# musket-ml/segmentation_training_pipeline

Hardware: AMD Instinct MI355X
Metric: images/sec U-Net/ResNet34 512x512 bs16 training step (higher is better)
Workload: dtype bf16; 1 GPU; U-Net/ResNet34 512x512x3 1-class, batch 16 per GPU, BCE+Dice, Adam, on-device augment S1 (BASELINE.json configs[1]); global_batch=16, parallelism=dp1, hipgraph=True

## Files before the change

### include/stp_hip.h

```cpp
#ifndef STP_HIP_H
#define STP_HIP_H

#include <stddef.h>
#include <stdint.h>

#ifdef __cplusplus
extern "C" {
#endif

#define STP_OK 0
#define STP_E_BADARG (-1)
#define STP_E_LAUNCH (-2)
#define STP_E_WORKSPACE (-3)

#define STP_F32 0
#define STP_BF16 1
#define STP_F16 3

#define STP_SRC_DIRECT 0
#define STP_SRC_NEAREST2X 1
#define STP_SRC_ZEROINS2X 2

int stp_abi_version(void);
int stp_storage_dtype(void);
// ... 83 lines not shown
  const float* src_bn_gamma;
  const float* src_bn_beta;
  int32_t src_bn_relu;
} stp_wgrad_params;

size_t stp_conv2d_wgrad_workspace_bytes(const stp_wgrad_params* p);
int stp_conv2d_wgrad(const stp_wgrad_params* p, void* workspace, size_t workspace_bytes, void* stream);
int stp_conv2d_wgrad_partial(const stp_wgrad_params* p, void* workspace, size_t workspace_bytes, int32_t variant, void* stream);
int stp_conv2d_wgrad_reduce(const stp_wgrad_params* p, const void* workspace, int32_t variant, void* stream);
int stp_wgrad_sc_eligible(const stp_wgrad_params* p);
int stp_wgrad_sc_slabs(const stp_wgrad_params* p);
int stp_wgrad_sc_partial(const stp_wgrad_params* p, void* workspace, void* stream);
int stp_conv2d_wgrad_kernel_id(const stp_wgrad_params* p);

int stp_wgrad_group_class(const stp_wgrad_params* p);
size_t stp_wgrad_group_table_bytes(const stp_wgrad_params* const* layers, int32_t n);
size_t stp_wgrad_group_workspace_bytes(const stp_wgrad_params* const* layers, int32_t n);
int stp_wgrad_group_build(const stp_wgrad_params* const* layers, int32_t n, void* host_table, size_t table_bytes);
int stp_wgrad_group_partial(const void* host_table, const void* dev_table, void* workspace, size_t workspace_bytes, void* stream);
int stp_wgrad_group_reduce(const void* host_table, const void* dev_table, const void* workspace, void* stream);

int stp_weight_prepare(const float* master, void* fwd, void* bwd, int32_t Cout, int32_t KH, int32_t KW,
                       int32_t Cin, int32_t KWp, int32_t Cinp, int32_t CoutB, int32_t dtype, void* stream);
size_t stp_weight_prepare_desc_bytes(void);
int64_t stp_weight_prepare_desc_fill(void* desc_host, int32_t index, int64_t start, const float* master, void* fwd, void* bwd,
                                     int32_t Cout, int32_t KH, int32_t KW, int32_t Cin, int32_t KWp, int32_t Cinp, int32_t CoutB);
int stp_weight_prepare_batched(const void* desc_dev, int32_t nlayers, int64_t total, int32_t dtype, void* stream);
int stp_weight_grad_unpad(const float* padded, float* grad, int32_t Cout, int32_t KH, int32_t KW,
                          int32_t Cin, int32_t KWp, int32_t Cinp, int32_t accumulate, void* stream);
int stp_stem_beta_grad(const float* padded_dw, const float* master, float* dbeta, int32_t Cout, int32_t KH,
                       int32_t KW, int32_t Cin, int32_t KWp, int32_t Cinp, int32_t one_ch, void* stream);

#define STP_U8 2
size_t stp_bn_workspace_bytes(int32_t C);
int stp_bn_apply_slots(const void* x, void* y, int32_t dtype, int64_t rows, int32_t C, const int64_t* slots, int32_t nslots,
                       float eps, float momentum, float* mean, float* rstd, float* moving_mean, float* moving_var,
                       const float* gamma, const float* beta, int32_t relu, void* stream);
int stp_bn_backward_slots(const void* x, const void* g, void* dx, int32_t dtype, int64_t rows, int32_t C, const float* mean,
                          const float* rstd, const float* gamma, const int64_t* slots, int32_t nslots, float* dgamma,
                          float* dbeta, int32_t accumulate_dx, void* stream);
int stp_zero_bytes(void* p, int64_t bytes, void* stream);
int stp_bn_backward_fused(const void* x, const void* g, void* dx, int32_t dtype, int64_t rows, int32_t C,
                          const float* mean, const float* rstd, const float* gamma, const float* partial, int32_t tiles,
                          float* dgamma, float* dbeta, int32_t accumulate_dx, void* workspace, size_t workspace_bytes,
                          void* stream);
int stp_bn_finalize_apply_ok(int32_t dtype, int64_t rows, int32_t C, int32_t tiles);
int stp_bn_finalize_apply(const float* partial, int32_t tiles, const void* x, void* y, int32_t dtype, int64_t rows, int32_t C,
                          float eps, float momentum, float* mean, float* rstd, float* moving_mean, float* moving_var,
                          const float* gamma, const float* beta, int32_t relu, void* stream);
int stp_bn_backward_fused_add(const void* x, const void* g, void* dx, const void* dadd, int32_t dtype, int64_t rows, int32_t C,
                              const float* mean, const float* rstd, const float* gamma, const float* partial, int32_t tiles,
                              float* dgamma, float* dbeta, int32_t accumulate_dx, void* workspace, size_t workspace_bytes,
                              void* stream);
int stp_bn_stats(const void* x, int32_t xdtype, int64_t rows, int32_t C, float eps, float momentum,
                 float* mean, float* rstd, float* moving_mean, float* moving_var,
                 void* workspace, size_t workspace_bytes, void* stream);
int stp_bn_finalize(const float* partial, int32_t tiles, int64_t rows, int32_t C, float eps, float momentum,
                    float* mean, float* rstd, float* moving_mean, float* moving_var, void* stream);
int stp_bn_apply(const void* x, int32_t xdtype, void* y, int32_t ydtype, int64_t rows, int32_t C, int32_t Cy,
                 const float* mean, const float* rstd, const float* gamma, const float* beta,
                 int32_t relu, float pad_value, void* stream);
int stp_bn_inference(const void* x, int32_t xdtype, void* y, int32_t ydtype, int64_t rows, int32_t C, int32_t Cy,
                     const float* moving_mean, const float* moving_var, float eps,
                     const float* gamma, const float* beta, int32_t relu, float pad_value, void* stream);
int stp_bn_backward(const void* x, const void* dy, void* dx, int32_t dtype, int64_t rows, int32_t C,
                    const float* mean, const float* rstd, const float* gamma, const float* beta,
                    float* dgamma, float* dbeta, int32_t relu, int32_t accumulate_dx,
                    void* workspace, size_t workspace_bytes, void* stream);

int stp_maxpool3x3s2(const void* x, void* y, uint8_t* idx, int32_t N, int32_t H, int32_t W, int32_t C,
                     int32_t dtype, void* stream);
int stp_maxpool3x3s2_bwd(const uint8_t* idx, const void* dy, void* dx, int32_t N, int32_t H, int32_t W, int32_t C,
                         int32_t dtype, int32_t accumulate, void* stream);
int stp_bn_apply_maxpool3x3s2(const void* x, void* yb, void* y, uint8_t* idx, int32_t N, int32_t H, int32_t W, int32_t C, int32_t dtype,
                              const float* mean, const float* rstd, const float* gamma, const float* beta, int32_t relu, void* stream);
int stp_maxpool3x3s2_bwd_bn_tiles(int32_t N, int32_t H, int32_t W, int32_t C, int32_t dtype);
int stp_maxpool3x3s2_bwd_bn(const uint8_t* idx, const void* dy, void* dx, int32_t N, int32_t H, int32_t W, int32_t C, int32_t dtype,
                            int32_t accumulate, const void* bn_x, const float* mean, const float* rstd, const float* gamma,
                            const float* beta, int32_t relu, float* partial, void* stream);
int stp_maxpool2x2(const void* x, void* y, uint8_t* idx, int32_t N, int32_t H, int32_t W, int32_t C, int32_t dtype, void* stream);
int stp_maxpool2x2_bwd(const uint8_t* idx, const void* dy, void* dx, int32_t N, int32_t H, int32_t W, int32_t C, int32_t dtype,
                       int32_t accumulate, void* stream);
size_t stp_avgpool_workspace_bytes(int32_t N, int32_t H, int32_t W, int32_t C, int32_t k);
int stp_avgpool(const void* x, void* y, int32_t N, int32_t H, int32_t W, int32_t C, int32_t k, int32_t dtype, void* workspace,
                size_t workspace_bytes, void* stream);
int stp_avgpool_bwd(const void* dy, void* dx, int32_t N, int32_t H, int32_t W, int32_t C, int32_t k, int32_t dtype,
                    int32_t accumulate, void* stream);
int stp_avgpool_pyramid_ok(int32_t N, int32_t H, int32_t W, int32_t C, int32_t k0, int32_t k1, int32_t k2, int32_t k3, int32_t dtype);
size_t stp_avgpool_pyramid_workspace_bytes(int32_t N, int32_t H, int32_t W, int32_t C, int32_t k0, int32_t dtype);
int stp_avgpool_pyramid(const void* x, void* y0, void* y1, void* y2, void* y3, int32_t k0, int32_t k1, int32_t k2, int32_t k3, int32_t N,
                        int32_t H, int32_t W, int32_t C, int32_t dtype, void* workspace, size_t workspace_bytes, void* stream);
int stp_avgpool_pyramid_bwd(const void* dy0, const void* dy1, const void* dy2, const void* dy3, int32_t k0, int32_t k1, int32_t k2, int32_t k3,
                            void* dx, int32_t N, int32_t H, int32_t W, int32_t C, int32_t dtype, int32_t accumulate, void* stream);
int stp_maxpool_k(const void* x, void* y, int32_t* idx, int32_t N, int32_t H, int32_t W, int32_t C, int32_t k, int32_t dtype, void* stream);
int stp_maxpool_k_bwd(const int32_t* idx, const void* dy, void* dx, int32_t N, int32_t H, int32_t W, int32_t C, int32_t k, int32_t dtype,
                      int32_t accumulate, void* stream);
int stp_relu_bwd(const void* y, void* dy, int64_t count, int32_t dtype, void* stream);

int stp_upsample2x_bwd(const void* dy, void* dx, int32_t N, int32_t H, int32_t W, int32_t C, int32_t ldy,
                       int32_t dtype, int32_t accumulate, void* stream);
int stp_tapsum_fwd(const void* z, void* y, const float* bias, int32_t N, int32_t H, int32_t W, int32_t Cout, int32_t Zc, int32_t Cy, int32_t dtype,
                   void* stream);
int stp_tapsum_bwd(const void* dy, void* dz, int32_t N, int32_t H, int32_t W, int32_t Cout, int32_t Cdy, int32_t Cdz, int32_t dtype, void* stream);
int stp_scatter2x_bwd(const void* t, void* dx, int32_t N, int32_t H, int32_t W, int32_t C, int32_t dtype, int32_t accumulate, void* stream);
int stp_scatter2x_bwd_bn_tiles(int32_t N, int32_t H, int32_t W, int32_t C, int32_t dtype);
int stp_scatter2x_bwd_bn(const void* t, void* dx, int32_t N, int32_t H, int32_t W, int32_t C, int32_t dtype, int32_t accumulate,
// ... 225 lines not shown
```

### segmentation_training_pipeline_amd/_lib.py

```python
import ctypes as C
import os

HERE = os.path.dirname(os.path.abspath(__file__))
LIB_PATH = os.environ.get("STP_LIB") or os.path.join(HERE, "libstp_hip.so")

LIB_F16_PATH = os.environ.get("STP_LIB_F16") or os.path.join(HERE, "libstp_hip_f16.so")

F32, BF16, U8, F16 = 0, 1, 2, 3
SRC_DIRECT, SRC_NEAREST2X, SRC_ZEROINS2X = 0, 1, 2

vp, i32, i64, f32, sz = C.c_void_p, C.c_int32, C.c_int64, C.c_float, C.c_size_t


class StpError(RuntimeError):
    pass


class ConvParams(C.Structure):
    _fields_ = [("src0", vp), ("src1", vp), ("weight", vp), ("bias", vp), ("residual", vp), ("dst0", vp), ("dst1", vp),
                ("N", i32), ("Hs0", i32), ("Ws0", i32), ("Hv", i32), ("Wv", i32), ("C0", i32), ("C1", i32),
                ("src0_mode", i32), ("KH", i32), ("KW", i32), ("stride", i32), ("pad", i32),
                ("Ho", i32), ("Wo", i32), ("Cout", i32), ("Cd0", i32),
                ("accumulate0", i32), ("accumulate1", i32), ("relu", i32), ("dtype", i32), ("tile", i32),
                ("stats_tiles", i32), ("stats_partial", vp),
# ... 31 lines not shown
    "stp_conv2d_scw": (i32, [C.POINTER(ConvParams), vp]),
    "stp_conv2d_scw_eligible": (i32, [C.POINTER(ConvParams)]),
    "stp_conv2d_scw_stats_tiles": (i32, [C.POINTER(ConvParams)]),
    "stp_conv2d_scn": (i32, [C.POINTER(ConvParams), vp]),
    "stp_conv2d_scn_eligible": (i32, [C.POINTER(ConvParams)]),
    "stp_conv2d_scn_stats_tiles": (i32, [C.POINTER(ConvParams)]),
    "stp_conv2d_s64": (i32, [C.POINTER(ConvParams), vp]),
    "stp_conv2d_s64_eligible": (i32, [C.POINTER(ConvParams)]),
    "stp_conv2d_s64_stats_tiles": (i32, [C.POINTER(ConvParams)]),
    "stp_conv2d_pw_eligible": (i32, [C.POINTER(ConvParams)]),
    "stp_conv2d_pw_cols": (i32, [C.POINTER(ConvParams)]),
    "stp_conv2d_pw": (i32, [C.POINTER(ConvParams), vp]),
    "stp_conv2d_stem_eligible": (i32, [C.POINTER(ConvParams)]),
    "stp_conv2d_stem": (i32, [C.POINTER(ConvParams), vp]),
    "stp_conv2d_halo_variant": (i32, [C.POINTER(ConvParams)]),
    "stp_conv2d_halo_tiles": (i32, [C.POINTER(ConvParams), i32]),
    "stp_conv2d_halo": (i32, [C.POINTER(ConvParams), i32, vp]),
    "stp_conv2d_wgrad_workspace_bytes": (sz, [C.POINTER(WgradParams)]),
    "stp_conv2d_wgrad": (i32, [C.POINTER(WgradParams), vp, sz, vp]),
    "stp_conv2d_wgrad_partial": (i32, [C.POINTER(WgradParams), vp, sz, i32, vp]),
    "stp_conv2d_wgrad_reduce": (i32, [C.POINTER(WgradParams), vp, i32, vp]),
    "stp_wgrad_reduce_desc_bytes": (sz, []),
    "stp_wgrad_reduce_desc_fill": (i64, [vp, i32, C.POINTER(WgradParams), vp]),
    "stp_wgrad_reduce_batched": (i32, [vp, i32, i64, vp]),
    "stp_wgrad_sc_eligible": (i32, [C.POINTER(WgradParams)]),
    "stp_wgrad_sc_slabs": (i32, [C.POINTER(WgradParams)]),
    "stp_wgrad_sc_partial": (i32, [C.POINTER(WgradParams), vp, vp]),
    "stp_conv2d_wgrad_kernel_id": (i32, [C.POINTER(WgradParams)]),
    "stp_wgrad_group_class": (i32, [C.POINTER(WgradParams)]),
    "stp_wgrad_group_table_bytes": (sz, [vp, i32]),
    "stp_wgrad_group_workspace_bytes": (sz, [vp, i32]),
    "stp_wgrad_group_build": (i32, [vp, i32, vp, sz]),
    "stp_wgrad_group_partial": (i32, [vp, vp, vp, sz, vp]),
    "stp_wgrad_group_reduce": (i32, [vp, vp, vp, vp]),
    "stp_weight_prepare": (i32, [vp, vp, vp, i32, i32, i32, i32, i32, i32, i32, i32, vp]),
    "stp_weight_prepare_desc_bytes": (sz, []),
    "stp_weight_prepare_desc_fill": (i64, [vp, i32, i64, vp, vp, vp, i32, i32, i32, i32, i32, i32, i32]),
    "stp_weight_prepare_batched": (i32, [vp, i32, i64, i32, vp]),
    "stp_weight_grad_unpad": (i32, [vp, vp, i32, i32, i32, i32, i32, i32, i32, vp]),
    "stp_stem_beta_grad": (i32, [vp, vp, vp, i32, i32, i32, i32, i32, i32, i32, vp]),
    "stp_bn_workspace_bytes": (sz, [i32]),
    "stp_bn_stats": (i32, [vp, i32, i64, i32, f32, f32, vp, vp, vp, vp, vp, sz, vp]),
    "stp_bn_finalize": (i32, [vp, i32, i64, i32, f32, f32, vp, vp, vp, vp, vp]),
    "stp_bn_apply": (i32, [vp, i32, vp, i32, i64, i32, i32, vp, vp, vp, vp, i32, f32, vp]),
    "stp_bn_inference": (i32, [vp, i32, vp, i32, i64, i32, i32, vp, vp, f32, vp, vp, i32, f32, vp]),
    "stp_bn_backward": (i32, [vp, vp, vp, i32, i64, i32, vp, vp, vp, vp, vp, vp, i32, i32, vp, sz, vp]),
    "stp_bn_apply_slots": (i32, [vp, vp, i32, i64, i32, vp, i32, f32, f32, vp, vp, vp, vp, vp, vp, i32, vp]),
    "stp_bn_backward_slots": (i32, [vp, vp, vp, i32, i64, i32, vp, vp, vp, vp, i32, vp, vp, i32, vp]),
    "stp_zero_bytes": (i32, [vp, i64, vp]),
    "stp_bn_backward_fused": (i32, [vp, vp, vp, i32, i64, i32, vp, vp, vp, vp, i32, vp, vp, i32, vp, sz, vp]),
    "stp_bn_finalize_apply_ok": (i32, [i32, i64, i32, i32]),
    "stp_bn_finalize_apply": (i32, [vp, i32, vp, vp, i32, i64, i32, f32, f32, vp, vp, vp, vp, vp, vp, i32, vp]),
    "stp_bn_backward_fused_add": (i32, [vp, vp, vp, vp, i32, i64, i32, vp, vp, vp, vp, i32, vp, vp, i32, vp, sz, vp]),
    "stp_maxpool3x3s2": (i32, [vp, vp, vp, i32, i32, i32, i32, i32, vp]),
    "stp_maxpool3x3s2_bwd": (i32, [vp, vp, vp, i32, i32, i32, i32, i32, i32, vp]),
    "stp_bn_apply_maxpool3x3s2": (i32, [vp, vp, vp, vp, i32, i32, i32, i32, i32, vp, vp, vp, vp, i32, vp]),
    "stp_maxpool3x3s2_bwd_bn_tiles": (i32, [i32, i32, i32, i32, i32]),
    "stp_maxpool3x3s2_bwd_bn": (i32, [vp, vp, vp, i32, i32, i32, i32, i32, i32, vp, vp, vp, vp, vp, i32, vp, vp]),
    "stp_maxpool2x2": (i32, [vp, vp, vp, i32, i32, i32, i32, i32, vp]),
    "stp_maxpool2x2_bwd": (i32, [vp, vp, vp, i32, i32, i32, i32, i32, i32, vp]),
    "stp_avgpool_workspace_bytes": (sz, [i32, i32, i32, i32, i32]),
    "stp_avgpool": (i32, [vp, vp, i32, i32, i32, i32, i32, i32, vp, sz, vp]),
    "stp_avgpool_bwd": (i32, [vp, vp, i32, i32, i32, i32, i32, i32, i32, vp]),
    "stp_avgpool_pyramid_ok": (i32, [i32, i32, i32, i32, i32, i32, i32, i32, i32]),
    "stp_avgpool_pyramid_workspace_bytes": (sz, [i32, i32, i32, i32, i32, i32]),
    "stp_avgpool_pyramid": (i32, [vp, vp, vp, vp, vp, i32, i32, i32, i32, i32, i32, i32, i32, i32, vp, sz, vp]),
    "stp_avgpool_pyramid_bwd": (i32, [vp, vp, vp, vp, i32, i32, i32, i32, vp, i32, i32, i32, i32, i32, i32, vp]),
    "stp_maxpool_k": (i32, [vp, vp, vp, i32, i32, i32, i32, i32, i32, vp]),
    "stp_maxpool_k_bwd": (i32, [vp, vp, vp, i32, i32, i32, i32, i32, i32, i32, vp]),
    "stp_relu_bwd": (i32, [vp, vp, i64, i32, vp]),
    "stp_upsample2x_bwd": (i32, [vp, vp, i32, i32, i32, i32, i32, i32, i32, vp]),
    "stp_tapsum_fwd": (i32, [vp, vp, vp, i32, i32, i32, i32, i32, i32, i32, vp]),
    "stp_tapsum_bwd": (i32, [vp, vp, i32, i32, i32, i32, i32, i32, i32, vp]),
    "stp_scatter2x_bwd": (i32, [vp, vp, i32, i32, i32, i32, i32, i32, vp]),
    "stp_scatter2x_bwd_bn_tiles": (i32, [i32, i32, i32, i32, i32]),
    "stp_scatter2x_bwd_bn": (i32, [vp, vp, i32, i32, i32, i32, i32, i32, vp, vp, vp, vp, vp, i32, vp, vp]),
    "stp_upsample2x_bwd_bn_tiles": (i32, [i32, i32, i32, i32, i32, i32]),
    "stp_upsample2x_bwd_bn": (i32, [vp, vp, i32, i32, i32, i32, i32, i32, i32, vp, vp, vp, vp, vp, i32, vp, vp]),
    "stp_upsample2x_add": (i32, [vp, vp, i32, i32, i32, i32, i32, vp]),
    "stp_resize_bilinear": (i32, [vp, vp, i32, i32, i32, i32, i32, i32, i32, i32, vp]),
    "stp_upsample_sum": (i32, [vp, vp, vp, vp, i32, i32, i32, i32, vp, i32, i32, i32, i32, i32, vp]),
    "stp_copy_cols_f32": (i32, [vp, i32, vp, i32, i32, i32, i32, vp]),
    "stp_resize_bilinear_bwd_workspace_bytes": (sz, [i32, i32, i32, i32, i32]),
    "stp_resize_bilinear_bwd": (i32, [vp, vp, i32, i32, i32, i32, i32, i32, i32, i32, i32, vp, sz, vp]),
    "stp_resize_nearest": (i32, [vp, vp, i32, i32, i32, i32, i32, i32, i32, i32, vp]),
    "stp_resize_nearest_bwd": (i32, [vp, vp, i32, i32, i32, i32, i32, i32, i32, i32, i32, vp]),
    "stp_channel_sum": (i32, [vp, i32, i64, i32, vp, i32, vp, sz, vp]),
    "stp_add_inplace": (i32, [vp, vp, i64, i32, vp]),
    "stp_loss_workspace_bytes": (sz, []),
    "stp_sigmoid_bce_dice": (i32, [vp, vp, i64, i32, f32, f32, vp, vp, i32, f32, vp, sz, vp]),
    "stp_sigmoid_loss_ex": (i32, [vp, vp, i64, i32, vp, vp, vp, i32, f32, vp, sz, vp]),
    "stp_sigmoid_loss_bias_grad": (i32, [vp, i64, vp, i32, vp]),
    "stp_sigmoid_multilabel_loss": (i32, [vp, vp, i64, i32, i32, i32, vp, vp, vp, i32, f32, vp, sz, vp]),
    "stp_sigmoid_multilabel_bias_grad": (i32, [vp, i64, i32, vp, i32, vp]),
    "stp_softmax_loss_ex": (i32, [vp, vp, i64, i32, i32, i32, vp, vp, vp, i32, f32, vp, sz, vp]),
    "stp_softmax_loss_masked": (i32, [vp, vp, i64, i32, i32, i32, vp, vp, vp, i32, f32, vp, sz, i32, vp, vp]),
    "stp_lovasz_workspace_bytes": (sz, [i64, i32]),
    "stp_lovasz_hinge": (i32, [vp, vp, i32, i64, i32, f32, vp, vp, i32, vp, sz, vp]),
    "stp_sigmoid": (i32, [vp, vp, i64, i32, vp]),
    "stp_softmax_cce_dice": (i32, [vp, vp, i64, i32, i32, i32, f32, f32, vp, vp, i32, f32, vp, sz, vp]),
    "stp_softmax_cce_dice_up_ok": (i32, [i32, i32, i32]),
    "stp_softmax_cce_dice_up_corner_bytes": (sz, [i32, i32, i32, i32]),
    "stp_softmax_cce_dice_up": (i32, [vp, vp, i32, i32, i32, i32, i32, i32, i32, f32, f32, vp, vp, i32, f32, vp, vp, vp, sz, vp, sz, vp]),
    "stp_softmax": (i32, [vp, vp, i64, i32, i32, i32, vp]),
    "stp_class_confusion_workspace_bytes": (sz, [i32]),
    "stp_class_confusion": (i32, [vp, vp, i64, i32, i32, i32, vp, vp, sz, vp]),
# ... 132 lines not shown
```

### segmentation_training_pipeline_amd/csrc/bn_pool.hip

```cpp
#include "common.h"
#include <algorithm>
#include <cstdlib>

#define BN_MAX_BLOCKS 1024
#ifndef POOL_ROWS
#define POOL_ROWS 4
#endif


template <typename T> __device__ __forceinline__ f32x4 ld4(const T* p);
template <> __device__ __forceinline__ f32x4 ld4<float>(const float* p) { return load4(p); }
template <> __device__ __forceinline__ f32x4 ld4<bf16_t>(const bf16_t* p) { return load4(p); }

template <typename T, int V> __device__ __forceinline__ void ldv(const T* p, float (&o)[V]) {
  if constexpr (V == 4) {
    const f32x4 v = ld4<T>(p);
    o[0] = v.x; o[1] = v.y; o[2] = v.z; o[3] = v.w;
  } else {
    const u32x4 r = *reinterpret_cast<const u32x4*>(p);
#pragma unroll
    for (int e = 0; e < 4; ++e) { o[2 * e] = h16lo_to_f32(r[e]); o[2 * e + 1] = h16hi_to_f32(r[e]); }
  }
}
template <typename T, int V> __device__ __forceinline__ void stv(T* p, const float (&o)[V]) {
// ... 1014 lines not shown
      const float xhl = (xl - mu[2 * e]) * rs[2 * e], xhh = (xh_ - mu[2 * e + 1]) * rs[2 * e + 1];
      float ol = sc[2 * e] * (gl - k1[2 * e] - xhl * k2[2 * e]), oh = sc[2 * e + 1] * (gh - k1[2 * e + 1] - xhh * k2[2 * e + 1]);
      if (dadd) { ol += h16lo_to_f32(dr[e]); oh += h16hi_to_f32(dr[e]); }
      o[e] = pack_bf16x2(ol, oh);
    }
    *reinterpret_cast<u32x4*>(dx + off) = o;
  };
  if (pre) {
#pragma unroll
    for (int k = 0; k < 4; ++k) one((size_t)(r + 32 * k) * C + col, px[k], pg[k], pd[k]);
    r += 128;
  }
  for (; r + 96 < rb; r += 128) {
    u32x4 vx[4], vg[4], vd[4] = {z4, z4, z4, z4};
#pragma unroll
    for (int k = 0; k < 4; ++k) {
      const size_t o = (size_t)(r + 32 * k) * C + col;
      vx[k] = *reinterpret_cast<const u32x4*>(x + o);
      vg[k] = *reinterpret_cast<const u32x4*>(g + o);
      if (dadd) vd[k] = *reinterpret_cast<const u32x4*>(dadd + o);
    }
#pragma unroll
    for (int k = 0; k < 4; ++k) one((size_t)(r + 32 * k) * C + col, vx[k], vg[k], vd[k]);
  }
  for (; r < rb; r += 32) {
    const size_t o = (size_t)r * C + col;
    const u32x4 vx = *reinterpret_cast<const u32x4*>(x + o), vg = *reinterpret_cast<const u32x4*>(g + o);
    const u32x4 vd = dadd ? *reinterpret_cast<const u32x4*>(dadd + o) : z4;
    one(o, vx, vg, vd);
  }
}

static int bn_bwd_fused_launch(const void* x, const void* g, void* dx, const void* dadd, int64_t rows, int C, const float* mean, const float* rstd,
                               const float* gamma, const float* partial, int tiles, float* dgamma, float* dbeta, int accumulate_dx, hipStream_t s) {
  const int chunks = bn_fused_chunks(rows, C);
  hipLaunchKernelGGL(bn_bwd_finalize_apply_kernel, dim3((C / BNF_SLAB) * chunks), dim3(256), 0, s, partial, tiles, (const bf16_t*)x, (const bf16_t*)g,
                     (bf16_t*)dx, accumulate_dx ? (const bf16_t*)dadd : (const bf16_t*)nullptr, rows, C, chunks, (float)(1.0 / (double)rows), mean, rstd,
                     gamma, dgamma, dbeta);
  STP_LAUNCH_CHECK();
  return STP_OK;
}

__global__ __launch_bounds__(256) void bn_bwd_finalize_tiles_kernel(const float* __restrict__ partial, int tiles, int C, float* sums,
                                                                    float* dgamma, float* dbeta) {
  __shared__ double sh[2][4];
  const int c = blockIdx.x;
  double S, Q;
  bnf_channel_sums(partial + (size_t)c * tiles, partial + ((size_t)C + c) * tiles, tiles, sh, S, Q);
  if (threadIdx.x != 0) return;
  sums[c] = (float)S;
  sums[C + c] = (float)Q;
  if (dbeta) dbeta[c] = (float)S;
  if (dgamma) dgamma[c] = (float)Q;
}

extern "C" int stp_bn_backward_slots(const void* x, const void* g, void* dx, int32_t dtype, int64_t rows, int32_t C, const float* mean,
                                     const float* rstd, const float* gamma, const int64_t* slots, int32_t nslots, float* dgamma,
                                     float* dbeta, int32_t accumulate_dx, void* stream) {
  if (!stp_dtype_ok(dtype)) return STP_E_BADARG;
  if (!x || !g || !dx || !mean || !rstd || !slots || rows <= 0 || C <= 0 || (C & 3) || nslots < 1 || (nslots & (nslots - 1))) return STP_E_BADARG;
  hipStream_t s = (hipStream_t)stream;
  const bool v8 = dtype == STP_H16 && (C & 7) == 0;
  const size_t lds2 = 6 * (size_t)C * sizeof(float);
  const int gr = grid_fixed_channels(grid_for_amortised(rows * (C / (v8 ? 8 : 4)), 8), C / (v8 ? 8 : 4));
  const float inv_rows = (float)(1.0 / (double)rows);
  const long long* sl = (const long long*)slots;
  if (v8)
    hipLaunchKernelGGL((bn_bwd_apply_kernel<bf16_t, 8>), dim3(gr), dim3(256), lds2, s, (const bf16_t*)x, (const bf16_t*)g, (bf16_t*)dx, rows, C,
                       mean, rstd, gamma, (const float*)nullptr, (const float*)nullptr, inv_rows, 0, accumulate_dx, sl, nslots, dgamma, dbeta);
  else if (dtype == STP_H16)
    hipLaunchKernelGGL((bn_bwd_apply_kernel<bf16_t, 4>), dim3(gr), dim3(256), lds2, s, (const bf16_t*)x, (const bf16_t*)g, (bf16_t*)dx, rows, C,
                       mean, rstd, gamma, (const float*)nullptr, (const float*)nullptr, inv_rows, 0, accumulate_dx, sl, nslots, dgamma, dbeta);
  else if (dtype == STP_F32)
    hipLaunchKernelGGL((bn_bwd_apply_kernel<float, 4>), dim3(gr), dim3(256), lds2, s, (const float*)x, (const float*)g, (float*)dx, rows, C,
                       mean, rstd, gamma, (const float*)nullptr, (const float*)nullptr, inv_rows, 0, accumulate_dx, sl, nslots, dgamma, dbeta);
  else
    return STP_E_BADARG;
  STP_LAUNCH_CHECK();
  return STP_OK;
}

extern "C" int stp_bn_backward_fused_add(const void* x, const void* g, void* dx, const void* dadd, int32_t dtype, int64_t rows, int32_t C,
                                     const float* mean, const float* rstd, const float* gamma, const float* partial,
                                     int32_t tiles, float* dgamma, float* dbeta, int32_t accumulate_dx, void* workspace,
                                     size_t workspace_bytes, void* stream) {
  if (!stp_dtype_ok(dtype)) return STP_E_BADARG;
  if (!x || !g || !dx || (accumulate_dx && !dadd) || !mean || !rstd || !partial || !workspace || rows <= 0 || C <= 0 || (C & 3) || tiles <= 0) return STP_E_BADARG;
  if (workspace_bytes < stp_bn_workspace_bytes(C)) return STP_E_WORKSPACE;
  hipStream_t s = (hipStream_t)stream;
  if (bn_fused_ok(dtype, rows, C, tiles))
    return bn_bwd_fused_launch(x, g, dx, dadd, rows, C, mean, rstd, gamma, partial, tiles, dgamma, dbeta, accumulate_dx, s);
  float* sums = (float*)workspace + (size_t)(BN_MAX_BLOCKS - 1) * 2 * C;
  hipLaunchKernelGGL(bn_bwd_finalize_tiles_kernel, dim3(C), dim3(256), 0, s, partial, tiles, C, sums, dgamma, dbeta);
  STP_LAUNCH_CHECK();
  const bool v8 = dtype == STP_H16 && (C & 7) == 0;
  const size_t lds2 = 6 * (size_t)C * sizeof(float);
  const int gr = grid_fixed_channels(grid_for_amortised(rows * (C / (v8 ? 8 : 4)), 8), C / (v8 ? 8 : 4));
  const float inv_rows = (float)(1.0 / (double)rows);
  if (v8)
    hipLaunchKernelGGL((bn_bwd_apply_kernel<bf16_t, 8>), dim3(gr), dim3(256), lds2, s, (const bf16_t*)x, (const bf16_t*)g,
                       (bf16_t*)dx, rows, C, mean, rstd, gamma, (const float*)nullptr, sums, inv_rows, 0, accumulate_dx, (const long long*)nullptr, 0, (float*)nullptr, (float*)nullptr,
                       (const bf16_t*)dadd);
  else if (dtype == STP_H16)
    hipLaunchKernelGGL((bn_bwd_apply_kernel<bf16_t, 4>), dim3(gr), dim3(256), lds2, s, (const bf16_t*)x, (const bf16_t*)g,
                       (bf16_t*)dx, rows, C, mean, rstd, gamma, (const float*)nullptr, sums, inv_rows, 0, accumulate_dx, (const long long*)nullptr, 0, (float*)nullptr, (float*)nullptr,
                       (const bf16_t*)dadd);
// ... 1889 lines not shown
```

### segmentation_training_pipeline_amd/csrc/conv_sc.h

```cpp
#pragma once
#include "common.h"
#include <cstdlib>
#include <type_traits>
#include <utility>

struct ScArgs {
  const char* src;
  const char* weight;
  const float* bias;
  char* dst;
  int N, H, W, Hs, Ws, Cout, up, accumulate, relu;
  int tiles_x, tiles_y;
  FastDiv divTx, divTy;
  float* stats;
  int stat_slots;
  BnBack bnb;
  int sum2;
  uint32_t src_bytes;
  BnBack pbn;
};

template <typename T> struct ScStageBn;
template <> struct ScStageBn<float> {
  f32x4 sc, sh;
  __device__ __forceinline__ void load(const BnBack& b, int c) { const BnBackCh k = bnback_load(b, c); sc = k.sc; sh = k.sh; }
  __device__ __forceinline__ void load_tab(const float* tsc, const float* tsh, int c) {
    sc = *reinterpret_cast<const f32x4*>(tsc + c); sh = *reinterpret_cast<const f32x4*>(tsh + c);
  }
  __device__ __forceinline__ u32x4 apply(const u32x4& r, int relu) const {
    u32x4 o;
#pragma unroll
    for (int e = 0; e < 4; ++e) o[e] = __float_as_uint(bn_act(bn_affine(__uint_as_float(r[e]), sc[e], sh[e]), relu));
    return o;
  }
};
template <> struct ScStageBn<bf16_t> {
  f32x2 sc[4], sh[4];
  __device__ __forceinline__ void load(const BnBack& b, int c) {
    const BnBackCh k0 = bnback_load(b, c), k1 = bnback_load(b, c + 4);
    sc[0] = f32x2{k0.sc[0], k0.sc[1]}; sc[1] = f32x2{k0.sc[2], k0.sc[3]}; sc[2] = f32x2{k1.sc[0], k1.sc[1]}; sc[3] = f32x2{k1.sc[2], k1.sc[3]};
    sh[0] = f32x2{k0.sh[0], k0.sh[1]}; sh[1] = f32x2{k0.sh[2], k0.sh[3]}; sh[2] = f32x2{k1.sh[0], k1.sh[1]}; sh[3] = f32x2{k1.sh[2], k1.sh[3]};
  }
  __device__ __forceinline__ void load_tab(const float* tsc, const float* tsh, int c) {
#pragma unroll
    for (int e = 0; e < 4; ++e) { sc[e] = *reinterpret_cast<const f32x2*>(tsc + c + 2 * e); sh[e] = *reinterpret_cast<const f32x2*>(tsh + c + 2 * e); }
  }
  __device__ __forceinline__ u32x4 apply(const u32x4& r, int relu) const {
    u32x4 o;
#pragma unroll
    for (int e = 0; e < 4; ++e) {
      f32x2 v = {h16lo_to_f32(r[e]), h16hi_to_f32(r[e])};
      v = __builtin_elementwise_fma(v, sc[e], sh[e]);
      o[e] = pack_bf16x2(bn_act(v.x, relu), bn_act(v.y, relu));
    }
    return o;
  }
};


constexpr int SC_TH = 8, SC_TW = 32, SC_HW = SC_TW + 2, SC_HH = SC_TH + 2;

template <int... Ks, typename F>
__device__ __forceinline__ void sc_unroll_seq(std::integer_sequence<int, Ks...>, F&& f) { (f(std::integral_constant<int, Ks>{}), ...); }
template <int N, typename F>
__device__ __forceinline__ void sc_unroll(F&& f) { sc_unroll_seq(std::make_integer_sequence<int, N>{}, f); }
#ifndef SC_RING
#define SC_RING 8
#endif

#ifndef SC_WPE_SMALL
#define SC_WPE_SMALL 4
#endif

static inline bool sc_stream_on() {
  static const bool on = !(getenv("STP_SC_STREAM") && atoi(getenv("STP_SC_STREAM")) == 0);
  return on;
}
static inline int sc_cu_count() {
  static const int cus = [] {
    int d = 0, n = 0;
    if (hipGetDevice(&d) != hipSuccess || hipDeviceGetAttribute(&n, hipDeviceAttributeMultiprocessorCount, d) != hipSuccess || n <= 0) n = 256;
    return n;
  }();
  return cus;
}
static inline int sc_stream_blocks(int dtype, int cin, int cout, int ntiles) {
  const int per_cu = cout <= 16 ? (dtype == STP_H16 && cin <= 16 ? SC_WPE_SMALL : 3) : 2;
  const int64_t b = (int64_t)sc_cu_count() * per_cu;
  return (int)(b < ntiles ? b : ntiles);
}


struct ScWgArgs {
  const char* src;
  const char* dy;
  float* slabs;
  int N, H, W, Hs, Ws, Cout, up;
  int tiles_x, tiles_y, ntiles;
  int ctot, coff;
  uint32_t src_bytes, dy_bytes;
  BnBack pbn;
};

constexpr int ST_HH = (SC_TH - 1) * 2 + 7, ST_HW = 70, ST_WROW = 464, ST_HALO = ST_HH * ST_HW * 8, ST_WBYTES = 64 * ST_WROW;

struct StemArgs {
  const char* src;
  const char* weight;
  char* dst;
  int N, H, W, Ho, Wo, tiles_x, tiles_y;
  FastDiv divTx, divTy;
  float* stats;
  uint32_t src_bytes;
};

bool stem_lean_serves(int N, int H, int W);
int stem_lean_blocks(int ntiles);
int stem_lean_launch(const StemArgs& a, hipStream_t s);
bool stem_wg_lean_serves(int N, int H, int W, int Ho, int Wo);
int stem_wg_lean_blocks(int N, int Ho, int Wo);
int stem_wg_lean_launch(const void* src, const void* dy, float* slabs, int N, int H, int W, int Ho, int Wo, hipStream_t s);

int sc_lean_launch(const ScArgs& a, int cin, int dtype, hipStream_t s);
int sc_wg_lean_launch(const ScWgArgs& a, int cin, int cout, int dtype, int blocks, hipStream_t s);
```

### segmentation_training_pipeline_amd/csrc/conv_sc.hip

```cpp
#include "conv_sc.h"

__device__ __forceinline__ f32x4 sc_stored(f32x4 v, const float*) { return v; }
__device__ __forceinline__ f32x4 sc_stored(f32x4 v, const bf16_t*) {
  const uint32_t a = pack_bf16x2(v.x, v.y), b = pack_bf16x2(v.z, v.w);
  return f32x4{h16lo_to_f32(a), h16hi_to_f32(a), h16lo_to_f32(b), h16hi_to_f32(b)};
}

template <typename T> struct ScMma;
template <> struct ScMma<bf16_t> {
  __device__ static __forceinline__ void run(const u32x4& a, const u32x4& b, f32x4& c) {
    c = mfma16_16x16x32(a, b, c);
  }
};
template <> struct ScMma<float> {
  __device__ static __forceinline__ void run(const u32x4& a, const u32x4& b, f32x4& c) {
    c = __builtin_amdgcn_mfma_f32_16x16x4f32(__uint_as_float(a.x), __uint_as_float(b.x), c, 0, 0, 0);
    c = __builtin_amdgcn_mfma_f32_16x16x4f32(__uint_as_float(a.y), __uint_as_float(b.y), c, 0, 0, 0);
    c = __builtin_amdgcn_mfma_f32_16x16x4f32(__uint_as_float(a.z), __uint_as_float(b.z), c, 0, 0, 0);
    c = __builtin_amdgcn_mfma_f32_16x16x4f32(__uint_as_float(a.w), __uint_as_float(b.w), c, 0, 0, 0);
  }
};

template <typename T> struct ScRaw4;
template <> struct ScRaw4<float> {
// ... 481 lines not shown
  ep.reset_stats();
  for (int tile = t_first; tile < t_end; tile += 2 * t_step) {
    body(tile, std::integral_constant<int, 0>{});
    if (tile + t_step < t_end) body(tile + t_step, std::integral_constant<int, 1>{});
  }
  ep.flush_stats(a, red, (int)blockIdx.x, (int)gridDim.x, tid, wave, lr, lg);
}

template <typename T, int CIN, int TM>
static int launch_sc(const ScArgs& a, hipStream_t s) {
  const int ntiles = a.N * a.tiles_x * a.tiles_y;
  if (sc_stream_on()) {
    constexpr int NV = SC_HH * SC_HW * (CIN / Elem<T>::VEC), NPASS = (NV + 255) / 256;
    const size_t lds = (size_t)2 * NPASS * 4096 + (4 * TM * 16 * 2 + 128 + 64) * sizeof(float);
    const int blocks = sc_stream_blocks(Elem<T>::DTYPE, CIN, TM * 16, ntiles);
    static bool attr_set = false;
    if (lds > 64 * 1024 && !attr_set) {
      if (hipFuncSetAttribute(reinterpret_cast<const void*>(conv_sc_stream_kernel<T, CIN, TM>), hipFuncAttributeMaxDynamicSharedMemorySize, (int)lds) != hipSuccess)
        return STP_E_LAUNCH;
      attr_set = true;
    }
    hipLaunchKernelGGL((conv_sc_stream_kernel<T, CIN, TM>), dim3(blocks), dim3(256), lds, s, a);
    STP_LAUNCH_CHECK();
    return STP_OK;
  }
  const size_t lds = (size_t)SC_HH * SC_HW * CIN * sizeof(T) + 4 * TM * 16 * 2 * sizeof(float);
  hipLaunchKernelGGL((conv_sc_kernel<T, CIN, TM>), dim3(ntiles), dim3(256), lds, s, a);
  STP_LAUNCH_CHECK();
  return STP_OK;
}

extern "C" int stp_conv2d_sc_stats_tiles(const stp_conv_params* p) {
  const int ntiles = p->N * ceil_div(p->Hv, SC_TH) * ceil_div(p->Wv, SC_TW);
  if (!sc_stream_on() || p->stats_slots) return ntiles;
  return sc_stream_blocks(p->dtype, p->C0, p->Cout <= 16 ? 16 : 32, ntiles);
}

template <typename T>
static int dispatch_sc(const ScArgs& a, int cin, hipStream_t s) {
  const int tm = a.Cout <= 16 ? 1 : 2;
  switch (cin * 4 + tm) {
    case 4 * 4 + 1: if constexpr (sizeof(T) == 4) return launch_sc<T, 4, 1>(a, s); else return STP_E_BADARG;
    case 4 * 4 + 2: if constexpr (sizeof(T) == 4) return launch_sc<T, 4, 2>(a, s); else return STP_E_BADARG;
    case 8 * 4 + 1: return launch_sc<T, 8, 1>(a, s);
    case 8 * 4 + 2: return launch_sc<T, 8, 2>(a, s);
    case 16 * 4 + 1: return launch_sc<T, 16, 1>(a, s);
    case 16 * 4 + 2: return launch_sc<T, 16, 2>(a, s);
    case 32 * 4 + 1: return launch_sc<T, 32, 1>(a, s);
    case 32 * 4 + 2: return launch_sc<T, 32, 2>(a, s);
    default: return STP_E_BADARG;
  }
}

extern "C" int stp_conv2d_sc_eligible(const stp_conv_params* p) {
  if (!p || !stp_dtype_ok(p->dtype)) return 0;
  const int vec = p->dtype == STP_H16 ? 8 : 4;
  const int cin = p->C0;
  const bool cin_ok = p->dtype == STP_F32 ? (cin == 4 || cin == 8 || cin == 16) : (cin == 8 || cin == 16 || cin == 32);
  return p->KH == 3 && p->KW == 3 && p->stride == 1 && p->pad == 1 && p->C1 == 0 && cin_ok && (cin % vec) == 0 && p->Cout <= 32 &&
         p->Cd0 == p->Cout && !p->residual && p->Ho == p->Hv && p->Wo == p->Wv &&
         (p->src0_mode == STP_SRC_DIRECT || (p->src0_mode == STP_SRC_NEAREST2X && p->Hv == 2 * p->Hs0 && p->Wv == 2 * p->Ws0));
}

extern "C" int stp_conv2d_sc(const stp_conv_params* p, void* stream) {
  if (!stp_conv2d_sc_eligible(p) || !p->src0 || !p->weight || !p->dst0) return STP_E_BADARG;
  ScArgs a;
  a.src = (const char*)p->src0; a.weight = (const char*)p->weight; a.bias = p->bias; a.dst = (char*)p->dst0;
  a.N = p->N; a.H = p->Hv; a.W = p->Wv; a.Hs = p->Hs0; a.Ws = p->Ws0; a.Cout = p->Cout;
  a.up = p->src0_mode == STP_SRC_NEAREST2X; a.accumulate = p->accumulate0; a.relu = p->relu;
  {
    const uint64_t sb = (uint64_t)p->N * p->Hs0 * p->Ws0 * p->C0 * (p->dtype == STP_H16 ? 2 : 4);
    if (sb >= 0x80000000ull) return STP_E_BADARG;
    a.src_bytes = (uint32_t)sb;
  }
  a.tiles_x = ceil_div(a.W, SC_TW); a.tiles_y = ceil_div(a.H, SC_TH);
  a.divTx = make_fastdiv((uint32_t)a.tiles_x); a.divTy = make_fastdiv((uint32_t)a.tiles_y);
  a.stats = p->stats_partial;
  a.stat_slots = p->stats_slots;
  if (a.stats && (p->Cout & 3)) return STP_E_BADARG;
  if (a.stat_slots && (!a.stats || (a.stat_slots & (a.stat_slots - 1)) || a.stat_slots > 64)) return STP_E_BADARG;
  a.bnb.x = (const char*)p->bnb_x; a.bnb.mean = p->bnb_mean; a.bnb.rstd = p->bnb_rstd; a.bnb.gamma = p->bnb_gamma;
  a.bnb.beta = p->bnb_beta; a.bnb.relu = p->bnb_relu;
  a.sum2 = p->dst_sum2x2;
  a.pbn.x = nullptr; a.pbn.mean = p->src_bn_mean; a.pbn.rstd = p->src_bn_rstd; a.pbn.gamma = p->src_bn_gamma; a.pbn.beta = p->src_bn_beta;
  a.pbn.relu = p->src_bn_relu;
  if (a.pbn.mean && !a.pbn.rstd) return STP_E_BADARG;
  if (a.bnb.x && (!a.stats || !a.bnb.mean || !a.bnb.rstd || p->relu)) return STP_E_BADARG;
  if (a.sum2 && ((p->Cout & 3) || (a.H & 1) || (a.W & 1) || p->bias || p->relu || (a.stats && !a.bnb.x))) return STP_E_BADARG;
  const_cast<stp_conv_params*>(p)->stats_tiles = stp_conv2d_sc_stats_tiles(p);
  hipStream_t s = (hipStream_t)stream;
  {
    const int r = sc_lean_launch(a, p->C0, p->dtype, s);
    if (r != 1) return r;
  }
  return p->dtype == STP_H16 ? dispatch_sc<bf16_t>(a, p->C0, s) : dispatch_sc<float>(a, p->C0, s);
}

struct ScwArgs {
  const char* src;
  const char* weight;
  char* dst_up;
  char* dst_sk;
  int N, H, W, C0, C1, acc_up, acc_sk;
  int tiles_x, tiles_y;
  FastDiv divTx, divTy;
  float* stats;
  BnBack bnb;
  uint32_t src_bytes, x_bytes;
  uint32_t up_bytes, sk_bytes;
};

template <typename T>
__global__ __launch_bounds__(256, 2) void conv_scw_stream_kernel(const ScwArgs a) {
  constexpr int CIN = 32, SZ = (int)sizeof(T), K = 9 * CIN, NCH = 9, VPP = 4, PIXB = CIN * SZ;
  constexpr int NV = SC_HH * SC_HW * VPP, NPASS = (NV + 255) / 256, BUF = NPASS * 4096;
  static_assert(SZ == 2, "16-bit storage");
  extern __shared__ __attribute__((aligned(16))) char smem[];
  float* ktab = reinterpret_cast<float*>(smem + 2 * BUF);
  constexpr int XBUF = 3 * 4096;
  char* const xlds = smem + 2 * BUF + 2048;
  const int tid = threadIdx.x, lane = tid & 63;
  const int wave = __builtin_amdgcn_readfirstlane(tid >> 6);
  const int lr = lane & 15, lg = lane >> 4;
  const int cbi[2] = {a.C0 == 64 ? wave * 16 : wave * 32, a.C0 == 64 ? 64 + wave * 16 : wave * 32 + 16};
  const bool upi[2] = {cbi[0] < a.C0, cbi[1] < a.C0};

  const int ntiles = a.N * a.tiles_x * a.tiles_y;
  int t_first, t_step, t_end;
  if ((gridDim.x & 7) == 0) {
    const int q = ntiles >> 3, r = ntiles & 7, x = blockIdx.x & 7;
    const int start = x < r ? x * (q + 1) : r * (q + 1) + (x - r) * q;
    t_first = start + (int)(blockIdx.x >> 3); t_step = (int)(gridDim.x >> 3); t_end = start + q + (x < r ? 1 : 0);
  } else {
    t_first = (int)blockIdx.x; t_step = (int)gridDim.x; t_end = ntiles;
  }
  if (t_first >= t_end) {
    if (a.stats && tid < a.C0) {
      a.stats[(size_t)tid * gridDim.x + blockIdx.x] = 0.f;
      a.stats[((size_t)a.C0 + tid) * gridDim.x + blockIdx.x] = 0.f;
    }
    return;
  }

  const __amdgpu_buffer_rsrc_t rs = __builtin_amdgcn_make_buffer_rsrc((void*)a.src, 0, a.src_bytes, 0x00020000);
  const int H2 = a.H >> 1, W2 = a.W >> 1;
  const bool bnb = a.bnb.x != nullptr;
  const bool xrs_on = bnb;
  const __amdgpu_buffer_rsrc_t xrs = __builtin_amdgcn_make_buffer_rsrc((void*)(bnb ? a.bnb.x : a.src), 0, bnb ? a.x_bytes : 0u, 0x00020000);
// ... 1212 lines not shown
          const int x = s * 4 + lg;
          float fa[TMo];
#pragma unroll
          for (int i = 0; i < TMo; ++i) fa[i] = *reinterpret_cast<const float*>(dyt + ((row * SC_TW + x) * COUT + i * 16 + lr) * SZ);
#pragma unroll
          for (int t = 0; t < 3; ++t) {
            const int tap = wave + 4 * t;
            if (tap < 9) {
              const int kh = tap / 3, kw = tap - kh * 3;
#pragma unroll
              for (int j = 0; j < TNi; ++j) {
                const float fb = *reinterpret_cast<const float*>(halo + (((row + kh) * SC_HW + x + kw) * CIN + j * 16 + lr) * SZ);
#pragma unroll
                for (int i = 0; i < TMo; ++i) acc[t][i][j] = __builtin_amdgcn_mfma_f32_16x16x4f32(fa[i], fb, acc[t][i][j], 0, 0, 0);
              }
            }
          }
        }
      }
    }
  }

  float* out = a.slabs + (size_t)blockIdx.x * a.Cout * (9 * a.ctot);
#pragma unroll
  for (int t = 0; t < 3; ++t) {
    const int tap = wave + 4 * t;
    if (tap >= 9) continue;
#pragma unroll
    for (int i = 0; i < TMo; ++i)
#pragma unroll
      for (int j = 0; j < TNi; ++j)
#pragma unroll
        for (int r = 0; r < 4; ++r) {
          const int co = i * 16 + lg * 4 + r;
          if (co < a.Cout) out[(size_t)co * (9 * a.ctot) + tap * a.ctot + a.coff + j * 16 + lr] = acc[t][i][j][r];
        }
  }
}

#define SC_WG_MAX_BLOCKS 1024

static bool wgrad_stem_shape(const stp_wgrad_params* p) {
  return p->dtype == STP_H16 && p->C0 == 4 && p->C1 == 0 && p->KH == 7 && p->KW == 8 && p->stride == 2 && p->pad == 3 && p->Cout == 64 &&
         p->src0_mode == STP_SRC_DIRECT && p->Hs0 == p->Hv && p->Ws0 == p->Wv && p->Ho == (p->Hv - 1) / 2 + 1 && p->Wo == (p->Wv - 1) / 2 + 1 &&
         !p->src_bn_mean && stem_wg_lean_serves(p->N, p->Hv, p->Wv, p->Ho, p->Wo);
}

extern "C" int stp_wgrad_sc_eligible(const stp_wgrad_params* p) {
  if (!p || !stp_dtype_ok(p->dtype)) return 0;
  if (wgrad_stem_shape(p)) return 1;
  const int vec = p->dtype == STP_H16 ? 8 : 4;
  const bool c0ok = p->C0 == 16 || p->C0 == 32 || (p->C0 == 64 && vec == 8);
  const bool c1ok = p->C1 == 0 || p->C1 == 16 || p->C1 == 32 || (p->C1 == 64 && vec == 8);
  return p->KH == 3 && p->KW == 3 && p->stride == 1 && p->pad == 1 && c0ok && c1ok &&
         (p->Cout == 8 || p->Cout == 16 || p->Cout == 32 || (p->Cout == 4 && vec == 4)) && (p->Cout % vec) == 0 &&
         p->Ho == p->Hv && p->Wo == p->Wv &&
         (p->src0_mode == STP_SRC_DIRECT || (p->src0_mode == STP_SRC_NEAREST2X && p->Hv == 2 * p->Hs0 && p->Wv == 2 * p->Ws0));
}

extern "C" int stp_wgrad_sc_slabs(const stp_wgrad_params* p) {
  if (wgrad_stem_shape(p)) return stem_wg_lean_blocks(p->N, p->Ho, p->Wo);
  const int64_t tiles = (int64_t)p->N * ceil_div(p->Hv, SC_TH) * ceil_div(p->Wv, SC_TW);
  static const int max_blocks = getenv("STP_SC_WG_BLOCKS") ? atoi(getenv("STP_SC_WG_BLOCKS")) : SC_WG_MAX_BLOCKS;
  const int vec = p->dtype == STP_H16 ? 8 : 4, cin = p->C0 > p->C1 ? p->C0 : p->C1;
  const int64_t npx = ((int64_t)SC_HH * SC_HW * (cin / vec) + 255) / 256, npd = ((int64_t)SC_TH * SC_TW * ((p->Cout + vec - 1) / vec) + 255) / 256;
  const int64_t lds = 2 * (npx + npd) * 4096;
  int per_cu = (int)((160 * 1024) / (lds > 0 ? lds : 1));
  per_cu = per_cu < 1 ? 1 : per_cu > 4 ? 4 : per_cu;
  int64_t blocks = (int64_t)sc_cu_count() * per_cu;
  if (blocks > max_blocks) blocks = max_blocks;
  return (int)(tiles < blocks ? tiles : blocks);
}

template <typename T, int CIN, int COUT>
static int launch_sc_wg(const ScWgArgs& a, int blocks, hipStream_t s) {
  if (sc_stream_on() && a.src_bytes && a.dy_bytes) {
    constexpr int VEC = Elem<T>::VEC;
    constexpr int NPX = (SC_HH * SC_HW * (CIN / VEC) + 255) / 256, NPD = (SC_TH * SC_TW * (COUT / VEC) + 255) / 256;
    const size_t lds = (size_t)2 * (NPX + NPD) * 4096;
    static bool attr_set = false;
    if (lds > 64 * 1024 && !attr_set) {
      if (hipFuncSetAttribute(reinterpret_cast<const void*>(conv_sc_wgrad_stream_kernel<T, CIN, COUT>), hipFuncAttributeMaxDynamicSharedMemorySize, (int)lds) != hipSuccess)
        return STP_E_LAUNCH;
      attr_set = true;
    }
    hipLaunchKernelGGL((conv_sc_wgrad_stream_kernel<T, CIN, COUT>), dim3(blocks), dim3(256), lds, s, a);
    STP_LAUNCH_CHECK();
    return STP_OK;
  }
  const size_t lds = (size_t)SC_HH * SC_HW * CIN * sizeof(T) + (size_t)SC_TH * SC_TW * COUT * sizeof(T) + 64;
  hipLaunchKernelGGL((conv_sc_wgrad_kernel<T, CIN, COUT>), dim3(blocks), dim3(256), lds, s, a);
  STP_LAUNCH_CHECK();
  return STP_OK;
}

template <typename T>
static int sc_wg_dispatch(const ScWgArgs& a, int cin, int cout, int blocks, hipStream_t s) {
  {
    const int r = sc_wg_lean_launch(a, cin, cout, Elem<T>::DTYPE, blocks, s);
    if (r != 1) return r;
  }
  const int key = cin * 64 + cout;
  if constexpr (sizeof(T) == 2) {
    switch (key) {
      case 16 * 64 + 8: return launch_sc_wg<T, 16, 8>(a, blocks, s);
      case 16 * 64 + 16: return launch_sc_wg<T, 16, 16>(a, blocks, s);
// ... 51 lines not shown
```

### segmentation_training_pipeline_amd/csrc/conv_sc_lean.hip

```cpp
#include "conv_sc.h"

enum { SCL_STATS = 0, SCL_BNB = 1, SCL_BNB_SUM2 = 2, SCL_HEAD = 3 };

struct TileC { int n, y0, x0; bool interior; };

__device__ __forceinline__ f32x2 scl_unpack(uint32_t w) { return f32x2{h16lo_to_f32(w), h16hi_to_f32(w)}; }

template <int TM>
__device__ __forceinline__ void scl_store(char* p, const u32x2 (&o)[TM]) {
  if constexpr (TM == 2) *reinterpret_cast<u32x4*>(p) = u32x4{o[0].x, o[0].y, o[1].x, o[1].y};
  else *reinterpret_cast<u32x2*>(p) = o[0];
}

template <int CIN, int TM, int EPI, bool PBN, bool UP>
__global__ __launch_bounds__(256, (TM == 1 ? (CIN <= 16 ? SC_WPE_SMALL : 3) : 2)) void conv_sc_lean_kernel(const ScArgs a) {
  typedef bf16_t T;
  constexpr int SZ = 2, VEC = 8, KC = 32, K = 9 * CIN, NCH = (K + KC - 1) / KC, VPP = CIN / VEC, PIXB = CIN * SZ;
  constexpr int HH = UP ? SC_TH / 2 + 2 : SC_HH, HW = UP ? SC_TW / 2 + 2 : SC_HW;
  constexpr int NV = HH * HW * VPP, NPASS = (NV + 255) / 256, BUF = NPASS * 4096;
  constexpr bool PART = (K % KC) != 0;
  constexpr int COUT = EPI == SCL_HEAD ? 1 : TM * 16;
  constexpr int CB = COUT * SZ;
  static_assert(EPI != SCL_HEAD || TM == 1, "head: one output channel");
  static_assert(!PBN || EPI == SCL_STATS || EPI == SCL_HEAD, "producer BatchNormalization: forward only");

  extern __shared__ __attribute__((aligned(16))) char smem[];
  float* red = reinterpret_cast<float*>(smem + 2 * BUF);
  float* ptab = red + 4 * TM * 16 * 2;
  const int tid = threadIdx.x, lane = tid & 63;
  const int wave = __builtin_amdgcn_readfirstlane(tid >> 6);
  const int lr = lane & 15, lg = lane >> 4;
  constexpr int sh = UP ? 1 : 0;

  const int ntiles = a.N * a.tiles_x * a.tiles_y;
  int t_first, t_step, t_end;
  if ((gridDim.x & 7) == 0) {
    const int q = ntiles >> 3, r = ntiles & 7, x = blockIdx.x & 7;
    const int start = x < r ? x * (q + 1) : r * (q + 1) + (x - r) * q;
    t_first = start + (int)(blockIdx.x >> 3); t_step = (int)(gridDim.x >> 3); t_end = start + q + (x < r ? 1 : 0);
  } else {
    t_first = (int)blockIdx.x; t_step = (int)gridDim.x; t_end = ntiles;
  }
  if (t_first >= t_end) return;

  const __amdgpu_buffer_rsrc_t rs = __builtin_amdgcn_make_buffer_rsrc((void*)a.src, 0, a.src_bytes, 0x00020000);
  int hyx[NPASS];
  uint32_t lo[NPASS];
  const int cvb = (tid % VPP) * 16;
#pragma unroll
  for (int p = 0; p < NPASS; ++p) {
    const int v = p * 256 + tid, pix = v / VPP;
    const int hy = pix / HW, hx = pix - hy * HW;
    hyx[p] = v < NV ? (hy << 16 | hx) : -1;
    lo[p] = v < NV ? (uint32_t)(((hy - 1) * a.Ws + (hx - 1)) * PIXB + cvb) : 0x80000000u;
  }

  auto decode = [&](int tile) -> TileC {
    const int bq = (int)fdiv((uint32_t)tile, a.divTx);
    const int tx = tile - bq * a.tiles_x;
    const int n = (int)fdiv((uint32_t)bq, a.divTy);
    const int ty = bq - n * a.tiles_y;
    TileC t;
    t.n = n; t.y0 = ty * SC_TH; t.x0 = tx * SC_TW;
    t.interior = ty > 0 && tx > 0 && t.y0 + SC_TH < a.H && t.x0 + SC_TW < a.W;
    return t;
  };
  auto issue_tile = [&](const TileC& t, int b, bool live) -> uint32_t {
    uint32_t inside = 0;
    if (live && t.interior) {
      const uint32_t tb = (uint32_t)((t.n * a.Hs + (t.y0 >> sh)) * a.Ws + (t.x0 >> sh)) * (uint32_t)PIXB;
#pragma unroll
      for (int p = 0; p < NPASS; ++p)
        __builtin_amdgcn_raw_ptr_buffer_load_lds(rs, (__attribute__((address_space(3))) void*)(smem + b * BUF + p * 4096 + wave * 1024), 16, (int)(tb + lo[p]), 0, 0, 0);
      inside = (1u << NPASS) - 1u;
    } else {
#pragma unroll
      for (int p = 0; p < NPASS; ++p) {
        const int gy = (t.y0 >> sh) - 1 + (hyx[p] >> 16), gx = (t.x0 >> sh) - 1 + (hyx[p] & 0xffff);
        const bool ok = live && hyx[p] >= 0 && (unsigned)gy < (unsigned)a.Hs && (unsigned)gx < (unsigned)a.Ws;
        const uint32_t off = ok ? (uint32_t)((t.n * a.Hs + gy) * a.Ws + gx) * (uint32_t)PIXB + (uint32_t)cvb : 0x80000000u;
        inside |= ok ? (1u << p) : 0u;
        __builtin_amdgcn_raw_ptr_buffer_load_lds(rs, (__attribute__((address_space(3))) void*)(smem + b * BUF + p * 4096 + wave * 1024), 16, (int)off, 0, 0, 0);
      }
    }
    return inside;
  };

  TileC tc = decode(t_first);
  uint32_t inside_cur = issue_tile(tc, 0, true);

  u32x4 fa[TM][NCH];
  constexpr int NA = UP ? 2 : 1;
  uint32_t bla[NA][NCH];
#pragma unroll
  for (int c = 0; c < NCH; ++c) {
    const int k0 = c * KC + lg * VEC;
    const int tap = k0 / CIN, ch = k0 - tap * CIN;
    const int kh = tap / 3, kw = tap - kh * 3;
#pragma unroll
    for (int ar = 0; ar < NA; ++ar) {
      const int prow = UP ? wave + ((ar + kh + 1) >> 1) : wave * 2 + kh, pcol = UP ? ((lr + kw + 1) >> 1) : kw + lr;
      bla[ar][c] = (uint32_t)(uintptr_t)smem + ((k0 < K) ? (uint32_t)(((prow * HW + pcol) * CIN + ch) * SZ) : 0u);
    }
#pragma unroll
    for (int i = 0; i < TM; ++i) {
      u32x4 w = {0u, 0u, 0u, 0u};
      const int wrow = TM == 2 ? (lr >> 2) * 8 + i * 4 + (lr & 3) : i * 16 + lr;
      if (k0 < K) w = *reinterpret_cast<const u32x4*>(a.weight + ((size_t)wrow * K + k0) * SZ);
      fa[i][c] = w;
    }
  }
  const bool last_ok = (NCH - 1) * KC + lg * VEC < K;
  if (PBN && tid < CIN) {
    const float r = a.pbn.rstd[tid], sc = a.pbn.gamma ? r * a.pbn.gamma[tid] : r;
    ptab[tid] = sc;
    ptab[32 + tid] = (a.pbn.beta ? a.pbn.beta[tid] : 0.f) - a.pbn.mean[tid] * sc;
  }
  f32x2 ksc[TM][2], ksh[TM][2];
  float alo = 0.f, ahi = 0.f;
  if constexpr (EPI == SCL_BNB || EPI == SCL_BNB_SUM2) {
#pragma unroll
    for (int i = 0; i < TM; ++i) {
      const BnBackCh k = bnback_load(a.bnb, TM == 2 ? lg * 8 + i * 4 : i * 16 + lg * 4);
      ksc[i][0] = f32x2{k.sc[0], k.sc[1]}; ksc[i][1] = f32x2{k.sc[2], k.sc[3]};
      ksh[i][0] = f32x2{k.sh[0], k.sh[1]}; ksh[i][1] = f32x2{k.sh[2], k.sh[3]};
    }
    alo = a.bnb.relu ? __uint_as_float(1u) : -__builtin_inff();
    ahi = a.bnb.relu == 2 ? __uint_as_float(0x40bfffffu) : __builtin_inff();
  }
  float bias0 = 0.f;
  if constexpr (EPI == SCL_HEAD) bias0 = a.bias ? a.bias[0] : 0.f;
  constexpr int LB = TM == 2 ? 16 : 8;
  const uint32_t so = EPI == SCL_BNB_SUM2 ? (uint32_t)((wave * (a.W >> 1) + (lr >> 1)) * CB + lg * LB)
                      : EPI == SCL_HEAD   ? (uint32_t)(((wave * 2) * a.W + lr) * CB)
                                          : (uint32_t)(((wave * 2) * a.W + lr) * CB + lg * LB);
  f32x4 ss[TM], qq[TM];
#pragma unroll
  for (int i = 0; i < TM; ++i) { ss[i] = f32x4{0.f, 0.f, 0.f, 0.f}; qq[i] = f32x4{0.f, 0.f, 0.f, 0.f}; }
  lds_barrier();

  const bool own = !(lr & 1);
  auto prefetch = [&](const TileC& pt, const bool EDGE, u32x2 (&xo)[TM][4]) __attribute__((always_inline)) {
    if constexpr (EPI == SCL_BNB) {
      const char* xb = a.bnb.x + (((size_t)pt.n * a.H + pt.y0) * a.W + pt.x0) * CB;
#pragma unroll
      for (int f = 0; f < 4; ++f) {
        const char* xf = xb + (size_t)(((f >> 1) * a.W + (f & 1) * 16) * CB);
        const bool ok = !EDGE || (pt.y0 + wave * 2 + (f >> 1) < a.H && pt.x0 + (f & 1) * 16 + lr < a.W);
        if constexpr (TM == 2) {
          const u32x4 w4 = *reinterpret_cast<const u32x4*>(ok ? xf + so : a.bnb.x);
          xo[0][f] = u32x2{w4.x, w4.y}; xo[TM - 1][f] = u32x2{w4.z, w4.w};
        } else {
          xo[0][f] = *reinterpret_cast<const u32x2*>(ok ? xf + so : a.bnb.x);
        }
      }
    }
    if constexpr (EPI == SCL_BNB_SUM2) {
      const char* xb = a.bnb.x + (((size_t)pt.n * (a.H >> 1) + (pt.y0 >> 1)) * (a.W >> 1) + (pt.x0 >> 1)) * CB;
#pragma unroll
      for (int h2 = 0; h2 < 2; ++h2) {
        const char* xf = xb + (size_t)(h2 * 8 * CB);
        const bool ok = own && (!EDGE || (pt.y0 + wave * 2 < a.H && pt.x0 + h2 * 16 + lr < a.W));
        if constexpr (TM == 2) {
          const u32x4 w4 = *reinterpret_cast<const u32x4*>(ok ? xf + so : a.bnb.x);
          xo[0][h2] = u32x2{w4.x, w4.y}; xo[TM - 1][h2] = u32x2{w4.z, w4.w};
        } else {
          xo[0][h2] = *reinterpret_cast<const u32x2*>(ok ? xf + so : a.bnb.x);
        }
      }
    }
  };
  u32x2 xp[TM][4];
  constexpr bool AHEAD = (EPI == SCL_BNB || EPI == SCL_BNB_SUM2) && !(CIN == 32 && TM == 2 && EPI == SCL_BNB);
  if constexpr (AHEAD) {
    if (tc.interior) prefetch(tc, false, xp); else prefetch(tc, true, xp);
  }

  int cur = 0;
  for (int tile = t_first; tile < t_end; tile += t_step, cur ^= 1) {
    const TileC t = tc;
    ScStageBn<T> sbn;
    if (PBN) sbn.load_tab(ptab, ptab + 32, (tid % VPP) * VEC);
    __builtin_amdgcn_s_waitcnt(0x0f70);
    asm volatile("" ::: "memory");
    if (PBN) {
#pragma unroll
      for (int p0 = 0; p0 < NPASS; p0 += 3) {
        u32x4 v[3];
#pragma unroll
        for (int q = 0; q < 3; ++q)
          if (p0 + q < NPASS) v[q] = *reinterpret_cast<const u32x4*>(smem + cur * BUF + ((p0 + q) * 256 + tid) * 16);
#pragma unroll
        for (int q = 0; q < 3; ++q)
          if (p0 + q < NPASS && (inside_cur & (1u << (p0 + q))))
            *reinterpret_cast<u32x4*>(smem + cur * BUF + ((p0 + q) * 256 + tid) * 16) = sbn.apply(v[q], a.pbn.relu);
      }
    }
    lds_barrier();

    const bool edge = !t.interior;
    if constexpr (!AHEAD) {
      if (edge) prefetch(t, true, xp); else prefetch(t, false, xp);
    }
    const int next = tile + t_step;
    const bool live = next < t_end;
    if (live) tc = decode(next);
    inside_cur = issue_tile(tc, cur ^ 1, live);
    u32x2 xn[TM][4];
    if (AHEAD && live) {
      if (tc.interior) prefetch(tc, false, xn); else prefetch(tc, true, xn);
    }

    f32x4 acc[TM][4];
#pragma unroll
    for (int i = 0; i < TM; ++i)
#pragma unroll
      for (int f = 0; f < 4; ++f) acc[i][f] = f32x4{0.f, 0.f, 0.f, 0.f};
    {
      constexpr int R = 4 * NCH;
      constexpr int RING = (CIN == 32 && TM == 2 && EPI == SCL_BNB_SUM2) ? 4 : SC_RING;
      constexpr int D = RING < R ? RING : R;
      u32x4 ring[D];
      auto issue = [&ring, &bla](auto kc) {
        constexpr int k = decltype(kc)::value, F = k / NCH, c = k % NCH;
        constexpr int OFF = UP ? (F & 1) * 8 * PIXB : ((F >> 1) * SC_HW + (F & 1) * 16) * PIXB;
        asm volatile("ds_read_b128 %0, %1 offset:%2" : "=v"(ring[k % D]) : "v"(bla[UP ? (F >> 1) : 0][c]), "n"(OFF));
      };
      sc_unroll<D>(issue);
      sc_unroll<R>([&ring, &fa, &acc, &issue, last_ok](auto kc) {
        constexpr int k = decltype(kc)::value, F = k / NCH, c = k % NCH;
        constexpr int young = (R - 1 - k) < (D - 1) ? (R - 1 - k) : (D - 1);
        asm volatile("s_waitcnt lgkmcnt(%1)" : "+v"(ring[k % D]) : "n"(young));
        u32x4 v = ring[k % D];
        if (PART && c == NCH - 1 && !last_ok) v = u32x4{0u, 0u, 0u, 0u};
#pragma unroll
        for (int i = 0; i < TM; ++i) acc[i][F] = mfma16_16x16x32(fa[i][c], v, acc[i][F]);
        if constexpr (k + D < R) issue(std::integral_constant<int, k + D>{});
      });
    }

    auto epilogue = [&](const bool EDGE) __attribute__((always_inline)) {
      bool okf[4];
#pragma unroll
      for (int f = 0; f < 4; ++f) okf[f] = !EDGE || (t.y0 + wave * 2 + (f >> 1) < a.H && t.x0 + (f & 1) * 16 + lr < a.W);
      if constexpr (EPI == SCL_STATS) {
        char* ob = a.dst + (((size_t)t.n * a.H + t.y0) * a.W + t.x0) * CB;
        const bool st = a.stats != nullptr;
#pragma unroll
        for (int f = 0; f < 4; ++f) {
          char* of = ob + (size_t)(((f >> 1) * a.W + (f & 1) * 16) * CB);
          u32x2 o[TM];
#pragma unroll
          for (int i = 0; i < TM; ++i) {
            const f32x4 v = acc[i][f];
            o[i] = u32x2{pack_bf16x2(v.x, v.y), pack_bf16x2(v.z, v.w)};
            if (st && okf[f]) {
              const f32x2 s0 = scl_unpack(o[i].x), s1 = scl_unpack(o[i].y);
              const f32x4 sv = {s0.x, s0.y, s1.x, s1.y};
              ss[i] += sv;
              qq[i] += sv * sv;
            }
          }
          if (okf[f]) scl_store<TM>(of + so, o);
        }
      }
      if constexpr (EPI == SCL_HEAD) {
        char* ob = a.dst + (((size_t)t.n * a.H + t.y0) * a.W + t.x0) * CB;
#pragma unroll
        for (int f = 0; f < 4; ++f) {
          char* of = ob + (size_t)(((f >> 1) * a.W + (f & 1) * 16) * CB);
          const float x = acc[0][f][0] + bias0;
          if (lg == 0 && okf[f]) *reinterpret_cast<T*>(of + so) = (T)(pack_bf16x2(x, 0.f) & 0xffffu);
        }
      }
      if constexpr (EPI == SCL_BNB) {
        char* ob = a.dst + (((size_t)t.n * a.H + t.y0) * a.W + t.x0) * CB;
#pragma unroll
        for (int f = 0; f < 4; ++f) {
          char* of = ob + (size_t)(((f >> 1) * a.W + (f & 1) * 16) * CB);
          u32x2 oo[TM];
#pragma unroll
          for (int i = 0; i < TM; ++i) {
            const f32x4 v = acc[i][f];
            u32x2& o = oo[i];
#pragma unroll
            for (int e = 0; e < 2; ++e) {
              const uint32_t stw = pack_bf16x2(v[2 * e], v[2 * e + 1]);
              const f32x2 dy = scl_unpack(stw), xv = scl_unpack(xp[i][f][e]);
              const f32x2 tt = __builtin_elementwise_fma(xv, ksc[i][e], ksh[i][e]);
              const f32x2 g = {okf[f] && __builtin_amdgcn_fmed3f(tt.x, alo, ahi) == tt.x ? dy.x : 0.f,
                               okf[f] && __builtin_amdgcn_fmed3f(tt.y, alo, ahi) == tt.y ? dy.y : 0.f};
              ss[i][2 * e] += g.x; ss[i][2 * e + 1] += g.y;
              qq[i][2 * e] = fmaf(g.x, xv.x, qq[i][2 * e]); qq[i][2 * e + 1] = fmaf(g.y, xv.y, qq[i][2 * e + 1]);
              o[e] = pack_bf16x2(g.x, g.y);
            }
          }
          if (okf[f]) scl_store<TM>(of + so, oo);
        }
      }
      if constexpr (EPI == SCL_BNB_SUM2) {
        char* ob = a.dst + (((size_t)t.n * (a.H >> 1) + (t.y0 >> 1)) * (a.W >> 1) + (t.x0 >> 1)) * CB;
#pragma unroll
        for (int h2 = 0; h2 < 2; ++h2) {
          char* of = ob + (size_t)(h2 * 8 * CB);
          const bool mine = own && okf[h2];
          u32x2 oo[TM];
#pragma unroll
          for (int i = 0; i < TM; ++i) {
            f32x4 v = acc[i][h2] + acc[i][h2 + 2];
#pragma unroll
            for (int e = 0; e < 4; ++e)
              v[e] += __int_as_float(__builtin_amdgcn_update_dpp(0, __float_as_int(v[e]), 0xB1, 0xf, 0xf, true));
            u32x2& o = oo[i];
#pragma unroll
            for (int e = 0; e < 2; ++e) {
              const uint32_t stw = pack_bf16x2(v[2 * e], v[2 * e + 1]);
              const f32x2 dy = scl_unpack(stw), xv = scl_unpack(xp[i][h2][e]);
              const f32x2 tt = __builtin_elementwise_fma(xv, ksc[i][e], ksh[i][e]);
              const f32x2 g = {mine && __builtin_amdgcn_fmed3f(tt.x, alo, ahi) == tt.x ? dy.x : 0.f,
                               mine && __builtin_amdgcn_fmed3f(tt.y, alo, ahi) == tt.y ? dy.y : 0.f};
              ss[i][2 * e] += g.x; ss[i][2 * e + 1] += g.y;
              qq[i][2 * e] = fmaf(g.x, xv.x, qq[i][2 * e]); qq[i][2 * e + 1] = fmaf(g.y, xv.y, qq[i][2 * e + 1]);
              o[e] = pack_bf16x2(g.x, g.y);
            }
          }
          if (mine) scl_store<TM>(of + so, oo);
        }
      }
    };
    if (edge) epilogue(true); else epilogue(false);
    {
      const uint32_t flip = cur ? (uint32_t)(-BUF) : (uint32_t)BUF;
#pragma unroll
      for (int ar = 0; ar < NA; ++ar)
#pragma unroll
        for (int c = 0; c < NCH; ++c) bla[ar][c] += flip;
    }
    if constexpr (AHEAD) {
#pragma unroll
      for (int i = 0; i < TM; ++i)
#pragma unroll
        for (int f = 0; f < 4; ++f) xp[i][f] = xn[i][f];
    }
  }

  if (EPI != SCL_HEAD && a.stats) {
    if constexpr (EPI == SCL_BNB || EPI == SCL_BNB_SUM2) {
#pragma unroll
      for (int i = 0; i < TM; ++i) {
        const int cb = TM == 2 ? lg * 8 + i * 4 : i * 16 + lg * 4;
        const f32x4 mu = *reinterpret_cast<const f32x4*>(a.bnb.mean + cb), rsd = *reinterpret_cast<const f32x4*>(a.bnb.rstd + cb);
#pragma unroll
        for (int e = 0; e < 4; ++e) qq[i][e] = rsd[e] * (qq[i][e] - mu[e] * ss[i][e]);
      }
    }
#pragma unroll
    for (int i = 0; i < TM; ++i)
#pragma unroll
      for (int e = 0; e < 4; ++e) {
        const float sv = row_sum16_to_lane15(ss[i][e]), qv = row_sum16_to_lane15(qq[i][e]);
        if (lr == 15) {
          const int cl = (TM == 2 ? lg * 8 + i * 4 : i * 16 + lg * 4) + e;
          red[(wave * TM * 16 + cl) * 2] = sv;
          red[(wave * TM * 16 + cl) * 2 + 1] = qv;
        }
      }
    lds_barrier();
    if (tid < TM * 16) {
      float sv = 0.f, qv = 0.f;
#pragma unroll
      for (int w = 0; w < 4; ++w) { sv += red[(w * TM * 16 + tid) * 2]; qv += red[(w * TM * 16 + tid) * 2 + 1]; }
      a.stats[(size_t)tid * gridDim.x + blockIdx.x] = sv;
      a.stats[((size_t)COUT + tid) * gridDim.x + blockIdx.x] = qv;
    }
  }
}

template <int CIN, int TM, int EPI, bool PBN, bool UP>
static int launch_scl(const ScArgs& a, hipStream_t s) {
  const int ntiles = a.N * a.tiles_x * a.tiles_y;
  constexpr int NV = (UP ? (SC_TH / 2 + 2) * (SC_TW / 2 + 2) : SC_HH * SC_HW) * (CIN / 8), NPASS = (NV + 255) / 256;
  const size_t lds = (size_t)2 * NPASS * 4096 + (4 * TM * 16 * 2 + 64) * sizeof(float);
  const int blocks = sc_stream_blocks(STP_H16, CIN, TM * 16, ntiles);
  static bool attr_set = false;
  if (lds > 64 * 1024 && !attr_set) {
    if (hipFuncSetAttribute(reinterpret_cast<const void*>(conv_sc_lean_kernel<CIN, TM, EPI, PBN, UP>), hipFuncAttributeMaxDynamicSharedMemorySize, (int)lds) != hipSuccess)
      return STP_E_LAUNCH;
    attr_set = true;
  }
  hipLaunchKernelGGL((conv_sc_lean_kernel<CIN, TM, EPI, PBN, UP>), dim3(blocks), dim3(256), lds, s, a);
  STP_LAUNCH_CHECK();
  return STP_OK;
}

template <int EPI, bool PBN, bool UP>
static int dispatch_scl2(const ScArgs& a, int cin, int tm, hipStream_t s) {
  switch (cin * 4 + tm) {
    case 8 * 4 + 1: return launch_scl<8, 1, EPI, PBN, UP>(a, s);
    case 16 * 4 + 1: return launch_scl<16, 1, EPI, PBN, UP>(a, s);
    case 32 * 4 + 1: return launch_scl<32, 1, EPI, PBN, UP>(a, s);
    case 8 * 4 + 2: if constexpr (EPI != SCL_HEAD) return launch_scl<8, 2, EPI, PBN, UP>(a, s); else return 1;
    case 16 * 4 + 2: if constexpr (EPI != SCL_HEAD) return launch_scl<16, 2, EPI, PBN, UP>(a, s); else return 1;
    case 32 * 4 + 2: if constexpr (EPI != SCL_HEAD) return launch_scl<32, 2, EPI, PBN, UP>(a, s); else return 1;
    default: return 1;
  }
}
template <int EPI, bool PBN>
static int dispatch_scl(const ScArgs& a, int cin, int tm, hipStream_t s) {
  if (a.up) {
    if constexpr (EPI == SCL_STATS) return dispatch_scl2<EPI, PBN, true>(a, cin, tm, s); else return 1;
  }
  return dispatch_scl2<EPI, PBN, false>(a, cin, tm, s);
}

static bool sc_lean_on() {
  static const bool on = !(getenv("STP_SC_LEAN") && atoi(getenv("STP_SC_LEAN")) == 0);
  return on;
}

int sc_lean_launch(const ScArgs& a, int cin, int dtype, hipStream_t s) {
  if (!sc_lean_on() || !sc_stream_on() || dtype != STP_H16 || a.stat_slots || a.accumulate || a.relu) return 1;
  const bool pbn = a.pbn.mean != nullptr;
  const int tm = a.Cout <= 16 ? 1 : 2;
  if (a.bnb.x) {
    if (pbn || a.bias || !a.stats || a.Cout != tm * 16) return 1;
    return a.sum2 ? dispatch_scl<SCL_BNB_SUM2, false>(a, cin, tm, s) : dispatch_scl<SCL_BNB, false>(a, cin, tm, s);
  }
  if (a.sum2) return 1;
  if (a.Cout == 1) {
    if (a.stats) return 1;
    return pbn ? dispatch_scl<SCL_HEAD, true>(a, cin, 1, s) : dispatch_scl<SCL_HEAD, false>(a, cin, 1, s);
  }
  if (a.bias || a.Cout != tm * 16) return 1;
  return pbn ? dispatch_scl<SCL_STATS, true>(a, cin, tm, s) : dispatch_scl<SCL_STATS, false>(a, cin, tm, s);
}

template <int CIN, int COUT, bool PBN, bool UP>
__global__ __launch_bounds__(256) void conv_sc_wgrad_lean_kernel(const ScWgArgs a) {
  typedef bf16_t T;
  constexpr int SZ = 2, VEC = 8, TMo = (COUT + 15) / 16, TNi = CIN / 16, PIXB = CIN * SZ, DYB = COUT * SZ;
  constexpr int VPPX = CIN / VEC, VPPD = COUT / VEC;
  constexpr int HH = UP ? SC_TH / 2 + 2 : SC_HH, HW = UP ? SC_TW / 2 + 2 : SC_HW;
  constexpr int NVX = HH * HW * VPPX, NPX = (NVX + 255) / 256;
  constexpr int NVD = SC_TH * SC_TW * VPPD, NPD = (NVD + 255) / 256;
  constexpr int XBUF = NPX * 4096, DBUF = NPD * 4096, BUF = XBUF + DBUF;
  constexpr int F3 = 3 * TMo * TNi;
  static_assert(4 * F3 * 1024 <= 2 * BUF, "the final reduction of a filter row fits the (dead) staging buffers");

  extern __shared__ __attribute__((aligned(16))) char smem[];
  const int tid = threadIdx.x, lane = tid & 63;
  const int wave = __builtin_amdgcn_readfirstlane(tid >> 6);
  const int lr = lane & 15, lg = lane >> 4;
  constexpr int sh = UP ? 1 : 0;

  int t_first, t_step, t_end;
  if ((gridDim.x & 7) == 0) {
    const int q = a.ntiles >> 3, r = a.ntiles & 7, x = blockIdx.x & 7;
    const int start = x < r ? x * (q + 1) : r * (q + 1) + (x - r) * q;
    t_first = start + (int)(blockIdx.x >> 3); t_step = (int)(gridDim.x >> 3); t_end = start + q + (x < r ? 1 : 0);
  } else {
    t_first = (int)blockIdx.x; t_step = (int)gridDim.x; t_end = a.ntiles;
  }

  f32x4 acc[9][TMo][TNi];
#pragma unroll
  for (int t = 0; t < 9; ++t)
#pragma unroll
    for (int i = 0; i < TMo; ++i)
#pragma unroll
      for (int j = 0; j < TNi; ++j) acc[t][i][j] = f32x4{0.f, 0.f, 0.f, 0.f};

  if (t_first < t_end) {
    const __amdgpu_buffer_rsrc_t rsx = __builtin_amdgcn_make_buffer_rsrc((void*)a.src, 0, a.src_bytes, 0x00020000);
    const __amdgpu_buffer_rsrc_t rsd = __builtin_amdgcn_make_buffer_rsrc((void*)a.dy, 0, a.dy_bytes, 0x00020000);
    int hyx[NPX], pyx[NPD];
    uint32_t lox[NPX], lod[NPD];
    const uint32_t cvx = (uint32_t)(tid % VPPX) * 16u, cvd = (uint32_t)(tid % VPPD) * 16u;
#pragma unroll
    for (int p = 0; p < NPX; ++p) {
      const int v = p * 256 + tid, pix = v / VPPX;
      const int hy = pix / HW, hx = pix - hy * HW;
      hyx[p] = v < NVX ? (hy << 16 | hx) : -1;
      lox[p] = v < NVX ? (uint32_t)(((hy - 1) * a.Ws + (hx - 1)) * PIXB) + cvx : 0x80000000u;
    }
#pragma unroll
    for (int p = 0; p < NPD; ++p) {
      const int v = p * 256 + tid, pix = v / VPPD;
      const int py = pix / SC_TW, px = pix % SC_TW;
      pyx[p] = v < NVD ? (py << 16 | px) : -1;
      lod[p] = v < NVD ? (uint32_t)((py * a.W + px) * DYB) + cvd : 0x80000000u;
    }
    auto decode = [&](int tile) -> TileC {
      int b = tile;
      const int tx = b % a.tiles_x; b /= a.tiles_x;
      const int ty = b % a.tiles_y;
      TileC t;
      t.n = b / a.tiles_y; t.y0 = ty * SC_TH; t.x0 = tx * SC_TW;
      t.interior = ty > 0 && tx > 0 && t.y0 + SC_TH < a.H && t.x0 + SC_TW < a.W;
      return t;
    };
    auto issue_tile = [&](const TileC& t, int bsel, bool live) -> uint32_t {
      uint32_t inside = 0;
      char* xb = smem + bsel * BUF;
      if (live && t.interior) {
        const uint32_t tbx = (uint32_t)((t.n * a.Hs + (t.y0 >> sh)) * a.Ws + (t.x0 >> sh)) * (uint32_t)PIXB;
        const uint32_t tbd = (uint32_t)((t.n * a.H + t.y0) * a.W + t.x0) * (uint32_t)DYB;
#pragma unroll
        for (int p = 0; p < NPX; ++p)
          __builtin_amdgcn_raw_ptr_buffer_load_lds(rsx, (__attribute__((address_space(3))) void*)(xb + p * 4096 + wave * 1024), 16, (int)(tbx + lox[p]), 0, 0, 0);
#pragma unroll
        for (int p = 0; p < NPD; ++p)
          __builtin_amdgcn_raw_ptr_buffer_load_lds(rsd, (__attribute__((address_space(3))) void*)(xb + XBUF + p * 4096 + wave * 1024), 16, (int)(tbd + lod[p]), 0, 0, 0);
        inside = (1u << NPX) - 1u;
      } else {
#pragma unroll
        for (int p = 0; p < NPX; ++p) {
          const int gy = (t.y0 >> sh) - 1 + (hyx[p] >> 16), gx = (t.x0 >> sh) - 1 + (hyx[p] & 0xffff);
          const bool ok = live && hyx[p] >= 0 && (unsigned)gy < (unsigned)a.Hs && (unsigned)gx < (unsigned)a.Ws;
          const uint32_t off = ok ? (uint32_t)((t.n * a.Hs + gy) * a.Ws + gx) * (uint32_t)PIXB + cvx : 0x80000000u;
          inside |= ok ? (1u << p) : 0u;
          __builtin_amdgcn_raw_ptr_buffer_load_lds(rsx, (__attribute__((address_space(3))) void*)(xb + p * 4096 + wave * 1024), 16, (int)off, 0, 0, 0);
        }
#pragma unroll
        for (int p = 0; p < NPD; ++p) {
          const int gy = t.y0 + (pyx[p] >> 16), gx = t.x0 + (pyx[p] & 0xffff);
          const bool ok = live && pyx[p] >= 0 && gy < a.H && gx < a.W;
          const uint32_t off = ok ? (uint32_t)((t.n * a.H + gy) * a.W + gx) * (uint32_t)DYB + cvd : 0x80000000u;
          __builtin_amdgcn_raw_ptr_buffer_load_lds(rsd, (__attribute__((address_space(3))) void*)(xb + XBUF + p * 4096 + wave * 1024), 16, (int)off, 0, 0, 0);
        }
      }
      return inside;
    };

    TileC tc = decode(t_first);
    uint32_t inside_cur = issue_tile(tc, 0, true);
    ScStageBn<T> sbn;
    if (PBN) sbn.load(a.pbn, (tid % VPPX) * VEC);
    const int xl = lg * 4 + (lr >> 2), qb = (lr & 3) * 8;
    const uint32_t aA0 = (uint32_t)(uintptr_t)smem + (uint32_t)(XBUF + ((2 * wave * SC_TW + xl) * COUT) * SZ + qb);
    uint32_t aB0[3];
#pragma unroll
    for (int kw = 0; kw < 3; ++kw)
      aB0[kw] = (uint32_t)(uintptr_t)smem + (uint32_t)((UP ? (wave * HW + ((xl + kw + 1) >> 1)) : ((2 * wave) * HW + xl + kw)) * CIN * SZ + qb);

    int cur = 0;
    for (int tile = t_first; tile < t_end; tile += t_step, cur ^= 1) {
      __builtin_amdgcn_s_waitcnt(0x0f70);
      asm volatile("" ::: "memory");
      if (PBN) {
#pragma unroll
        for (int p0 = 0; p0 < NPX; p0 += 3) {
          u32x4 v[3];
#pragma unroll
          for (int q = 0; q < 3; ++q)
            if (p0 + q < NPX) v[q] = *reinterpret_cast<const u32x4*>(smem + cur * BUF + ((p0 + q) * 256 + tid) * 16);
#pragma unroll
          for (int q = 0; q < 3; ++q)
            if (p0 + q < NPX && (inside_cur & (1u << (p0 + q))))
              *reinterpret_cast<u32x4*>(smem + cur * BUF + ((p0 + q) * 256 + tid) * 16) = sbn.apply(v[q], a.pbn.relu);
        }
      }
      lds_barrier();
      const int next = tile + t_step;
      const bool live = next < t_end;
      if (live) tc = decode(next);
      inside_cur = issue_tile(tc, cur ^ 1, live);

      const uint32_t aA = aA0 + (uint32_t)(cur * BUF);
      uint32_t aB[3];
#pragma unroll
      for (int kw = 0; kw < 3; ++kw) aB[kw] = aB0[kw] + (uint32_t)(cur * BUF);
      u32x2 fa[2][TMo][2];
      u32x2 fb[2][3][TNi][2];
      sc_unroll<2 * TMo * 2>([&fa, aA](auto kc) {
        constexpr int k = decltype(kc)::value, r = k / (TMo * 2), i = (k / 2) % TMo, hl = k & 1;
        asm volatile("ds_read_b64_tr_b16 %0, %1 offset:%2" : "=v"(fa[r][i][hl]) : "v"(aA), "n"((r * SC_TW * COUT + i * 16 + hl * 16 * COUT) * SZ));
      });
      auto issue_b = [&fb, &aB](auto hc) {
        constexpr int h = decltype(hc)::value;
        sc_unroll<3 * TNi * 2>([&fb, &aB](auto kc) {
          constexpr int k = decltype(kc)::value, kw = k / (TNi * 2), j = (k / 2) % TNi, hl = k & 1;
          constexpr int OFF = UP ? ((((h + 1) >> 1) * HW + hl * 8) * CIN + j * 16) * SZ : ((h * HW + hl * 16) * CIN + j * 16) * SZ;
          asm volatile("ds_read_b64_tr_b16 %0, %1 offset:%2" : "=v"(fb[h & 1][kw][j][hl]) : "v"(aB[kw]), "n"(OFF));
        });
      };
      issue_b(std::integral_constant<int, 0>{});
      sc_unroll<4>([&](auto hc) {
        constexpr int h = decltype(hc)::value;
        if constexpr (h < 3) issue_b(std::integral_constant<int, h + 1>{});
        asm volatile("s_waitcnt lgkmcnt(%0)" ::"n"(h < 3 ? 3 * TNi * 2 : 0) : "memory");
        if constexpr (h == 0) {
#pragma unroll
          for (int r = 0; r < 2; ++r)
#pragma unroll
            for (int i = 0; i < TMo; ++i) { asm volatile("" : "+v"(fa[r][i][0])); asm volatile("" : "+v"(fa[r][i][1])); }
        }
#pragma unroll
        for (int kw = 0; kw < 3; ++kw)
#pragma unroll
          for (int j = 0; j < TNi; ++j) { asm volatile("" : "+v"(fb[h & 1][kw][j][0])); asm volatile("" : "+v"(fb[h & 1][kw][j][1])); }
#pragma unroll
        for (int r = 0; r < 2; ++r) {
          const int kh = h - r;
          if (kh < 0 || kh > 2) continue;
#pragma unroll
          for (int kw = 0; kw < 3; ++kw)
#pragma unroll
            for (int j = 0; j < TNi; ++j) {
              const u32x4 vb = {fb[h & 1][kw][j][0].x, fb[h & 1][kw][j][0].y, fb[h & 1][kw][j][1].x, fb[h & 1][kw][j][1].y};
#pragma unroll
              for (int i = 0; i < TMo; ++i) {
                const u32x4 va = {fa[r][i][0].x, fa[r][i][0].y, fa[r][i][1].x, fa[r][i][1].y};
                acc[kh * 3 + kw][i][j] = mfma16_16x16x32(va, vb, acc[kh * 3 + kw][i][j]);
              }
            }
        }
      });
    }
  }

  float* out = a.slabs + (size_t)blockIdx.x * a.Cout * (9 * a.ctot);
  f32x4* rbuf = reinterpret_cast<f32x4*>(smem);
  __builtin_amdgcn_s_waitcnt(0x0f70);
#pragma unroll
  for (int kh = 0; kh < 3; ++kh) {
    lds_barrier();
#pragma unroll
    for (int kw = 0; kw < 3; ++kw)
#pragma unroll
      for (int i = 0; i < TMo; ++i)
#pragma unroll
        for (int j = 0; j < TNi; ++j) rbuf[(wave * F3 + (kw * TMo + i) * TNi + j) * 64 + lane] = acc[kh * 3 + kw][i][j];
    lds_barrier();
    for (int f = wave; f < F3; f += 4) {
      const f32x4 s01 = rbuf[(0 * F3 + f) * 64 + lane] + rbuf[(1 * F3 + f) * 64 + lane];
      const f32x4 s23 = rbuf[(2 * F3 + f) * 64 + lane] + rbuf[(3 * F3 + f) * 64 + lane];
      const f32x4 v = s01 + s23;
      const int kw = f / (TMo * TNi), i = (f / TNi) % TMo, j = f % TNi;
#pragma unroll
      for (int r = 0; r < 4; ++r) {
        const int co = i * 16 + lg * 4 + r;
        if (co < a.Cout) out[(size_t)co * (9 * a.ctot) + (kh * 3 + kw) * a.ctot + a.coff + j * 16 + lr] = v[r];
      }
    }
  }
}

template <int CIN, int COUT, bool PBN, bool UP>
static int launch_scwl(const ScWgArgs& a, int blocks, hipStream_t s) {
  constexpr int NPX = ((UP ? (SC_TH / 2 + 2) * (SC_TW / 2 + 2) : SC_HH * SC_HW) * (CIN / 8) + 255) / 256, NPD = (SC_TH * SC_TW * (COUT / 8) + 255) / 256;
  const size_t lds = (size_t)2 * (NPX + NPD) * 4096;
  static bool attr_set = false;
  if (lds > 64 * 1024 && !attr_set) {
    if (hipFuncSetAttribute(reinterpret_cast<const void*>(conv_sc_wgrad_lean_kernel<CIN, COUT, PBN, UP>), hipFuncAttributeMaxDynamicSharedMemorySize, (int)lds) != hipSuccess)
      return STP_E_LAUNCH;
    attr_set = true;
  }
  hipLaunchKernelGGL((conv_sc_wgrad_lean_kernel<CIN, COUT, PBN, UP>), dim3(blocks), dim3(256), lds, s, a);
  STP_LAUNCH_CHECK();
  return STP_OK;
}

static bool sc_wg_lean_3232() {
  static const bool on = getenv("STP_SC_WG_LEAN_3232") && atoi(getenv("STP_SC_WG_LEAN_3232")) != 0;
  return on;
}

template <bool PBN, bool UP>
static int dispatch_scwl(const ScWgArgs& a, int cin, int cout, int blocks, hipStream_t s) {
  switch (cin * 64 + cout) {
    case 16 * 64 + 8: return launch_scwl<16, 8, PBN, UP>(a, blocks, s);
    case 16 * 64 + 16: return launch_scwl<16, 16, PBN, UP>(a, blocks, s);
    case 16 * 64 + 32: return launch_scwl<16, 32, PBN, UP>(a, blocks, s);
    case 32 * 64 + 8: return launch_scwl<32, 8, PBN, UP>(a, blocks, s);
    case 32 * 64 + 16: return launch_scwl<32, 16, PBN, UP>(a, blocks, s);
    case 32 * 64 + 32: if (UP || sc_wg_lean_3232()) return launch_scwl<32, 32, PBN, UP>(a, blocks, s); else return 1;
    default: return 1;
  }
}

int sc_wg_lean_launch(const ScWgArgs& a, int cin, int cout, int dtype, int blocks, hipStream_t s) {
  if (!sc_lean_on() || !sc_stream_on() || dtype != STP_H16 || !a.src_bytes || !a.dy_bytes) return 1;
  if (a.up) return a.pbn.mean ? dispatch_scwl<true, true>(a, cin, cout, blocks, s) : dispatch_scwl<false, true>(a, cin, cout, blocks, s);
  return a.pbn.mean ? dispatch_scwl<true, false>(a, cin, cout, blocks, s) : dispatch_scwl<false, false>(a, cin, cout, blocks, s);
}

constexpr int STL_VPR = 35, STL_NV = ST_HH * STL_VPR, STL_NPASS = (STL_NV + 255) / 256, STL_BUF = STL_NPASS * 4096, STL_ROW = STL_VPR * 16;
constexpr int STL_LDS = ST_WBYTES + 2 * STL_BUF + 4 * 64 * 2 * 4;

__global__ __launch_bounds__(256, 2) void conv_stem_lean_kernel(const StemArgs a) {
  constexpr int TM = 4, NCH = 7, K = 224, COUT = 64;
  extern __shared__ __attribute__((aligned(16))) char smem[];
  char* const wl = smem;
  char* const hb = smem + ST_WBYTES;
  float* const red = reinterpret_cast<float*>(smem + ST_WBYTES + 2 * STL_BUF);
  const int tid = threadIdx.x, lane = tid & 63;
  const int wave = __builtin_amdgcn_readfirstlane(tid >> 6);
  const int lr = lane & 15, lg = lane >> 4;

  const int ntiles = a.N * a.tiles_x * a.tiles_y;
  int t_first, t_step, t_end;
  if ((gridDim.x & 7) == 0) {
    const int q = ntiles >> 3, r = ntiles & 7, x = blockIdx.x & 7;
    const int start = x < r ? x * (q + 1) : r * (q + 1) + (x - r) * q;
    t_first = start + (int)(blockIdx.x >> 3); t_step = (int)(gridDim.x >> 3); t_end = start + q + (x < r ? 1 : 0);
  } else {
    t_first = (int)blockIdx.x; t_step = (int)gridDim.x; t_end = ntiles;
  }
  f32x4 ss[TM], qq[TM];
#pragma unroll
  for (int i = 0; i < TM; ++i) { ss[i] = f32x4{0.f, 0.f, 0.f, 0.f}; qq[i] = f32x4{0.f, 0.f, 0.f, 0.f}; }

  if (t_first < t_end) {
    const __amdgpu_buffer_rsrc_t rs = __builtin_amdgcn_make_buffer_rsrc((void*)a.src, 0, a.src_bytes, 0x00020000);
    int hyx[STL_NPASS];
    uint32_t lo[STL_NPASS];
#pragma unroll
    for (int p = 0; p < STL_NPASS; ++p) {
      const int v = p * 256 + tid, hy = v / STL_VPR, vx = v - hy * STL_VPR;
      hyx[p] = v < STL_NV ? (hy << 16 | vx) : -1;
      lo[p] = v < STL_NV ? (uint32_t)((hy * a.W + 2 * vx) * 8) : 0x80000000u;
    }
    auto decode = [&](int tile) -> TileC {
// ... 342 lines not shown
```

### segmentation_training_pipeline_amd/graph.py

```python
import os
import ctypes as C
from collections import OrderedDict

import numpy as np
import torch

from . import _lib, ops

_TD = {"bf16": torch.bfloat16, "fp16": torch.float16, "fp32": torch.float32}


class StpShapeError(ValueError):
    pass


def _rup(a, b):
    return (a + b - 1) // b * b


class DT(object):
    __slots__ = ("name", "N", "H", "W", "C", "buf", "grad", "_grad_ready", "grad_writes", "needs_grad", "gradC", "meta")

    def __init__(self, name, N, H, W, Cn, buf=None, needs_grad=False):
        self.name, self.N, self.H, self.W, self.C = name, N, H, W, Cn
# ... 18 lines not shown


class ParamInfo(object):
    __slots__ = ("name", "offset", "numel", "shape", "kind", "trainable", "pending_slices")

    def __init__(self, name, offset, shape, kind, trainable):
        self.name, self.offset, self.shape, self.kind, self.trainable = name, offset, tuple(shape), kind, trainable
        self.numel = int(np.prod(shape))
        self.pending_slices = 0

    @property
    def end(self):
        return self.offset + self.numel


class Plan(object):
    def __init__(self, batch, dtype="bf16", device="cuda", training=True, class_metrics=False):
        if dtype not in _TD:
            raise ValueError("dtype must be 'bf16', 'fp16' or 'fp32'")
        self.device = torch.device(device)
        if self.device.type == "cuda" and not torch.cuda.is_available():
            raise _lib.StpError("the HIP training path needs a GPU; there is no CPU fallback")
        self.lib = _lib.load("fp16" if dtype == "fp16" else "bf16")
        self.loss_scale = 1.0
        self.dls = None
        self.N = batch
        self.dtype = dtype
        self.tdt = _TD[dtype]
        self.cdt = {"bf16": ops.BF16, "fp16": ops.F16, "fp32": ops.F32}[dtype]
        self.vec = 4 if dtype == "fp32" else 8
        self.training = training
        self.params = OrderedDict()
        self.states = OrderedDict()
        self._poff = 0
        self._soff = 0
        self.dry = True
        self.frozen_prefixes = ()
        self._keep = []
        self.tensors = OrderedDict()
        self.P = self.G = self.S = None
        self.prep, self.fwd, self.bwd, self.opt = [], [], [], []
        self._tape = []
        self._goffs = []
        self.bwd_marks, self.bwd_monotone = [], True
        self._prep_layers = []
        self._upc_layers = []
        self._upc4_layers = []
        self._wg_ws_bytes = 0
        self._bn_ws_c = 4
        self.bn_momentum = 0.99
        self.fuse_bn_backward = os.environ.get("STP_FUSE_BN_BACKWARD", "1") != "0"
        self.fuse_bn_backward_last = os.environ.get("STP_FUSE_BN_BACKWARD_LAST", "1") != "0"
        self.fold_upsample_grad = os.environ.get("STP_FOLD_UPSAMPLE_GRAD", "1") != "0"
        self.wgrad_group_gflop = float(os.environ.get("STP_WGRAD_GROUP_GFLOP", "300"))
        self.wgrad_lone_group_gflop = float(os.environ.get("STP_WGRAD_LONE_GROUP_GFLOP", "600"))
        self.reduce_batch = int(os.environ.get("STP_WGRAD_REDUCE_BATCH", "0"))
        self._pending_reduces, self._pending_reduce_hi = [], 0
        self._wgroup, self._wgroup_cls, self._wgroup_flops, self._wgroup_hi = [], 0, 0.0, 0
        self._wgroup_reads = set()
        self.wgroups = []
        self._dw_ws_bytes = 0
        self.step_state = None
        self.bn_slots = os.environ.get("STP_BN_SLOTS", "0") == "1"
        self.fuse_bn_sc = os.environ.get("STP_FUSE_BN_SC", "1") != "0"
        self.fuse_bn_halo = os.environ.get("STP_FUSE_BN_HALO", "0") != "0" and os.environ.get("STP_HALO", "1") != "0"
        self.bn_slots_max_rows = int(os.environ.get("STP_BN_SLOTS_MAXROWS", "1073741824"))
        self._slot_need = 0
        self._slot_used = 0
        self.slot_arena = None
        self.loss_scalars = None
        self.class_metrics = bool(class_metrics)
        self.masked_loss = None
        self.class_weights = None
        self.class_counts = None
        self.inputs = {}

    def define(self, net_fn, share=None):
        self.dry = True
        net_fn(self)
        n = _rup(self._poff, 4)
        if share is not None:
            if [(k, v.offset, v.shape) for k, v in share.params.items()] != [(k, v.offset, v.shape) for k, v in self.params.items()] \
                    or list(share.states.items()) != list(self.states.items()):
                raise StpShapeError("plans that share weights must declare identical parameters")
            self.P, self.S, self.G = share.P, share.S, None
        else:
            self.P = torch.zeros(n, dtype=torch.float32, device=self.device)
            self.G = torch.zeros(n, dtype=torch.float32, device=self.device) if self.training else None
            self.S = torch.zeros(max(_rup(self._soff, 4), 4), dtype=torch.float32, device=self.device)
        self.mask = torch.ones(n, dtype=torch.uint8, device=self.device)
        self.ws_wgrad = torch.empty(max(self._wg_ws_bytes // 4, 4) + 4, dtype=torch.float32, device=self.device)
        self.ws_bn = torch.empty(ops.bn_workspace_bytes(_rup(self._bn_ws_c, 4)) // 4, dtype=torch.float32, device=self.device)
        self.ws_loss = torch.empty(ops.loss_workspace_bytes() // 4, dtype=torch.float32, device=self.device)
        self.ws_dw = torch.empty(max(self._dw_ws_bytes // 4, 4), dtype=torch.float32, device=self.device)
        if self.training and self.bn_slots and self._slot_need:
            self.slot_arena = torch.zeros(_rup(self._slot_need, 2), dtype=torch.int64, device=self.device)
        self.dry = False
        self._tape = []
        self._prep_layers = []
        self._upc_layers = []
        self._upc4_layers = []
        self.tensors = OrderedDict()
        net_fn(self)
        self._fuse_bn_finalize(self._fuse_bn_into_consumers())
        self._finish_prep()
        if self.training:
# ... 306 lines not shown
            self._emit(self.fwd, "stp_bn_inference", x.buf.data_ptr(), ops.U8, out.buf.data_ptr(), self.cdt, x.rows, x.C, Cp,
                       self._sptr(mm), self._sptr(mv), eps, None, self._pptr(beta), 0, 1.0)
        return out

    def input_cast(self, name, x):
        if x.C > 7:
            raise StpShapeError("input_cast handles up to 7 image channels")
        Cp = 4 if x.C <= 3 else 8
        out = self._new(name, x.H, x.W, Cp, False)
        out.meta["real_c"] = x.C
        if self.dry:
            return out
        zero, one = self._alloc((8,), torch.float32), self._alloc((8,), torch.float32)
        zero.zero_(); one.fill_(1.0)
        self._emit(self.fwd, "stp_bn_apply", x.buf.data_ptr(), ops.U8, out.buf.data_ptr(), self.cdt, x.rows, x.C, Cp,
                   zero.data_ptr(), one.data_ptr(), None, None, 0, 0.0)
        return out

    def bn(self, name, x, eps, relu=True, scale=True, momentum=None):
        Cn = x.C
        relu = int(relu)
        momentum = self.bn_momentum if momentum is None else float(momentum)
        gamma = self.param(name + "/gamma", (Cn,), "gamma") if scale else None
        beta = self.param(name + "/beta", (Cn,), "beta")
        mm = self.state(name + "/moving_mean", Cn, 0.0)
        mv = self.state(name + "/moving_variance", Cn, 1.0)
        out = self._new(name, x.H, x.W, Cn, x.needs_grad or beta.trainable)
        self._bn_ws_c = max(self._bn_ws_c, Cn)
        self._use(x)
        if self.dry:
            self._slot_need += 4 * Cn * self._nslots(Cn)
            return out
        gp = self._pptr(gamma) if gamma else None
        if not self.training:
            self._emit(self.fwd, "stp_bn_inference", x.buf.data_ptr(), self.cdt, out.buf.data_ptr(), self.cdt, x.rows, Cn, Cn,
                       self._sptr(mm), self._sptr(mv), eps, gp, self._pptr(beta), int(relu), 0.0)
            return out
        mean, rstd = self._alloc((Cn,), torch.float32), self._alloc((Cn,), torch.float32)
        table = x.meta.get("stats_table")
        slots = x.meta.get("stats_slots")
        if slots is not None:
            self._emit(self.fwd, "stp_bn_apply_slots", x.buf.data_ptr(), out.buf.data_ptr(), self.cdt, x.rows, Cn, slots[0], slots[1], eps,
                       momentum, mean.data_ptr(), rstd.data_ptr(), self._sptr(mm), self._sptr(mv), gp, self._pptr(beta), int(relu))
        elif table is not None:
            self._emit(self.fwd, "stp_bn_finalize", table[0].data_ptr(), table[1], x.rows, Cn, eps, momentum, mean.data_ptr(),
                       rstd.data_ptr(), self._sptr(mm), self._sptr(mv))
        else:
            self._emit(self.fwd, "stp_bn_stats", x.buf.data_ptr(), self.cdt, x.rows, Cn, eps, momentum, mean.data_ptr(),
                       rstd.data_ptr(), self._sptr(mm), self._sptr(mv), self.ws_bn.data_ptr(), self.ws_bn.numel() * 4)
        if slots is None:
            self._emit(self.fwd, "stp_bn_apply", x.buf.data_ptr(), self.cdt, out.buf.data_ptr(), self.cdt, x.rows, Cn, Cn,
                       mean.data_ptr(), rstd.data_ptr(), gp, self._pptr(beta), int(relu), 0.0)
        out.meta["bn"] = (x.buf.data_ptr(), mean.data_ptr(), rstd.data_ptr(), gp, self._pptr(beta), int(relu))
        if self.fuse_bn_sc and slots is None:
            out.meta["apply_rec"] = self.fwd[-1]
            out.meta["sc_consumers"], out.meta["halo_consumers"] = [], []

        def back():
            if not out.needs_grad or not out.grad_ready:
                return
            bslots = out.meta.get("bnb_slots")
            dadd = None
            if (x.needs_grad and x.grad_ready and x.grad is not None and x.grad.data_ptr() in self._wgroup_reads and bslots is None
                    and out.meta.get("bnb") is not None):
                dadd, x.grad = x.grad, None
            dx = self._gradbuf(x) if x.needs_grad else self._alloc((x.N, x.H, x.W, Cn))
            if bslots is not None:
                self._emit(self.bwd, "stp_bn_backward_slots", x.buf.data_ptr(), out.grad.data_ptr(), dx.data_ptr(), self.cdt, x.rows, Cn,
                           mean.data_ptr(), rstd.data_ptr(), gp, bslots[0], bslots[1], self._gptr(gamma) if gamma else None,
                           self._gptr(beta), int(x.grad_ready and x.needs_grad))
            elif out.meta.get("bnb") is not None:
                st, q = out.meta["bnb"]
                tiles = q if isinstance(q, int) else int(self.lib.stp_conv2d_stats_floats(C.byref(q))) // (2 * Cn)
                if dadd is not None:
                    self._emit(self.bwd, "stp_bn_backward_fused_add", x.buf.data_ptr(), out.grad.data_ptr(), dx.data_ptr(), dadd.data_ptr(),
                               self.cdt, x.rows, Cn, mean.data_ptr(), rstd.data_ptr(), gp, st.data_ptr(), tiles,
                               self._gptr(gamma) if gamma else None, self._gptr(beta), 1, self.ws_bn.data_ptr(), self.ws_bn.numel() * 4)
                else:
                    self._emit(self.bwd, "stp_bn_backward_fused", x.buf.data_ptr(), out.grad.data_ptr(), dx.data_ptr(), self.cdt,
                               x.rows, Cn, mean.data_ptr(), rstd.data_ptr(), gp, st.data_ptr(), tiles,
                               self._gptr(gamma) if gamma else None, self._gptr(beta), int(x.grad_ready and x.needs_grad),
                               self.ws_bn.data_ptr(), self.ws_bn.numel() * 4)
            else:
                self._emit(self.bwd, "stp_bn_backward", x.buf.data_ptr(), out.grad.data_ptr(), dx.data_ptr(), self.cdt, x.rows, Cn,
                           mean.data_ptr(), rstd.data_ptr(), gp, self._pptr(beta), self._gptr(gamma) if gamma else None,
                           self._gptr(beta), int(relu), int(x.grad_ready and x.needs_grad), self.ws_bn.data_ptr(), self.ws_bn.numel() * 4)
            if x.needs_grad:
                x.grad_ready = True

        self._tape.append(back)
        return out

    def _emit_bias_grad(self, dy, rows, gradC, Cout, b):
        tmp = self._alloc((gradC,), torch.float32)
        self._emit(self.bwd, "stp_channel_sum", dy.data_ptr(), self.cdt, rows, gradC, tmp.data_ptr(), 0, self.ws_bn.data_ptr(), self.ws_bn.numel() * 4)
        self._emit(self.bwd, "stp_weight_grad_unpad", tmp.data_ptr(), self._gptr(b), Cout, 1, 1, 1, 1, 1, 0)

    def conv3x3_taps(self, name, x, Cout, bias=False):
        cin = x.meta.get("real_c", x.C)
        z = self.conv(name + "_taps", x, 9 * Cout, 1, param_name=name, param_shape=(Cout, 3, 3, cin), cout_pad=64 if self.dtype != "fp32" else None)
        b = self.param(name + "/bias", (Cout,), "bias") if bias else None
        out = self._new(name, x.H, x.W, Cout, z.needs_grad or (b is not None and b.trainable))
        out.gradC = _rup(Cout, self.vec)
        if bias:
            self._bn_ws_c = max(self._bn_ws_c, out.gradC)
        self._use(z)
        if self.dry:
            return out
        self._emit(self.fwd, "stp_tapsum_fwd", z.buf.data_ptr(), out.buf.data_ptr(), self._pptr(b) if b is not None else None, self.N, x.H, x.W,
                   Cout, z.C, Cout, self.cdt)
        if not self.training:
            return out

        def back():
            if not out.grad_ready:
                return
            dy = out.grad
            if b is not None and b.trainable:
                self._emit_bias_grad(dy, out.rows, out.gradC, Cout, b)
            if z.needs_grad:
                self._emit(self.bwd, "stp_tapsum_bwd", dy.data_ptr(), self._gradbuf(z).data_ptr(), self.N, x.H, x.W, Cout, out.gradC, z.gradC, self.cdt)
                z.grad_ready = True

        self._tape.append(back)
        return out

    def conv(self, name, x, Cout, k, stride=1, pad=0, src1=None, upsample=False, bias=False, residual=None, bn_stats=False,
             transpose=False, relu=False, same_tf=False, fold_shortcut=None, param_name=None, param_shape=None, cout_pad=None,
             param_cols=None, flops_as=None):
        L = ConvLayer(self, name, x, Cout, k, stride, pad, src1, upsample, residual, transpose, relu, same_tf, fold_shortcut, param_cols)
        L.declare(param_name, param_shape, cout_pad, bias)
        if self.dry:
            return L.out
        L.forward(bn_stats, flops_as)
        if self.training:
            self._tape.append(L.backward)
        return L.out

    def add(self, name, y, skip):
        if (y.H, y.W, y.C) != (skip.H, skip.W, skip.C):
            raise StpShapeError("%s: cannot add %dx%dx%d and %dx%dx%d" % (name, y.H, y.W, y.C, skip.H, skip.W, skip.C))
        out = DT(name, self.N, y.H, y.W, y.C, y.buf, y.needs_grad or skip.needs_grad)
        out.gradC = y.gradC
        self.tensors[name] = out
        self._use(y, skip)
        if self.dry:
            return out
        self._emit(self.fwd, "stp_add_inplace", y.buf.data_ptr(), skip.buf.data_ptr(), y.rows * y.C, self.cdt)
        if not self.training:
            return out

        def back():
            if not out.needs_grad or not out.grad_ready:
                return
            dy = out.grad
            if y.needs_grad:
                y.grad, y.grad_ready = dy, True
            if skip.needs_grad:
                if not skip.grad_ready and skip.gradC == out.gradC:
                    skip.grad, skip.grad_ready = dy, True
                else:
                    self._emit(self.bwd, "stp_add_inplace", self._gradbuf(skip).data_ptr(), dy.data_ptr(), y.rows * out.gradC,
                               self.cdt)

        self._tape.append(back)
        return out

    def se(self, name, u, shortcut, reduction=16, bn_stats=True):
        if (u.H, u.W, u.C) != (shortcut.H, shortcut.W, shortcut.C) or u.gradC != u.C or shortcut.gradC != u.C:
            raise StpShapeError("%s: cannot gate %dx%dx%d onto a %dx%dx%d shortcut" % (name, u.H, u.W, u.C, shortcut.H, shortcut.W, shortcut.C))
        Cn, HW = u.C, u.H * u.W
        R = Cn // int(reduction)
        chunks = int(self.lib.stp_se_chunks(self.N, HW, Cn))
        if chunks < 1 or not 1 <= R <= 32:
            raise StpShapeError("%s: squeeze-and-excitation serves 16..512 channels in multiples of 8 with 1..32 hidden units (got %d / %d)"
                                % (name, Cn, R))
        w1 = self.param(name + "_fc1/kernel", (1, 1, Cn, R), "sekernel")
        b1 = self.param(name + "_fc1/bias", (R,), "bias")
        w2 = self.param(name + "_fc2/kernel", (1, 1, R, Cn), "sekernel")
        b2 = self.param(name + "_fc2/bias", (Cn,), "bias")
        out = self._new(name, u.H, u.W, Cn, u.needs_grad or shortcut.needs_grad or w1.trainable)
        self._use(u, shortcut)
        if self.dry:
            return out
        wsp, wsb = self._scratch(self.lib.stp_se_workspace_bytes(self.N, HW, Cn))
        z, s = self._alloc((self.N * Cn,), torch.float32), self._alloc((self.N * Cn,), torch.float32)
        h = self._alloc((_rup(self.N * R, 4),), torch.float32)
# ... 458 lines not shown
            if not (x.needs_grad and out.grad_ready):
                return
            acc = int(x.grad_ready)
            self._emit_grad_pass("stp_maxpool3x3s2_bwd", x, acc, (self.N, x.H, x.W, x.C, self.cdt),
                                 (idx.data_ptr(), out.grad.data_ptr(), self._gradbuf(x).data_ptr(), self.N, x.H, x.W, x.C, self.cdt, acc),
                                 os.environ.get("STP_FUSE_POOL_BN", "0") == "1")
            x.grad_ready = True

        if self.training:
            self._tape.append(back)
        return out

    def _emit_loss(self, name, logits, target, dims, weights, tail=()):
        dl = self._gradbuf(logits) if self.training else None
        if len(weights) == 5:
            self._loss_weights = (C.c_float * 5)(*weights)
            weights = (C.addressof(self._loss_weights),)
        else:
            weights = tuple(float(w) for w in weights)
        self._emit(self.fwd, name, logits.buf.data_ptr(), target.buf.data_ptr(), *dims, self.cdt, *weights, self.loss_scalars.data_ptr(),
                   dl.data_ptr() if dl is not None else None, logits.gradC, float(self.loss_scale), self.ws_loss.data_ptr(),
                   self.ws_loss.numel() * 4, *tail)
        if self.training and self.dls is not None:
            self._emit(self.fwd, "stp_scale_by_device", dl.data_ptr(), logits.rows * logits.gradC, self.cdt, self.dls.data_ptr(), self.dls.data_ptr() + 16)
        return dl

    def _emit_confusion(self, rows, target, factor=0, ignore_label=None):
        if not self.class_metrics:
            return
        classes = rows.C
        nb = int(self.lib.stp_class_confusion_workspace_bytes(classes))
        if nb <= 0:
            raise StpShapeError("class metrics need a head of 2..32 classes")
        self.class_counts = self._alloc((classes * classes,), torch.int32)
        ws = self._alloc((nb // 4,), torch.int32)
        if factor:
            self._emit(self.fwd, "stp_class_confusion_up", rows.buf.data_ptr(), target.buf.data_ptr(), self.N, rows.H, rows.W, factor, classes,
                       rows.C, self.cdt, self.class_counts.data_ptr(), ws.data_ptr(), nb)
        elif ignore_label is not None:
            self._emit(self.fwd, "stp_class_confusion_ignore", rows.buf.data_ptr(), target.buf.data_ptr(), rows.rows, classes, rows.C, self.cdt,
                       self.class_counts.data_ptr(), ws.data_ptr(), nb, int(ignore_label))
        else:
            self._emit(self.fwd, "stp_class_confusion", rows.buf.data_ptr(), target.buf.data_ptr(), rows.rows, classes, rows.C, self.cdt,
                       self.class_counts.data_ptr(), ws.data_ptr(), nb)

    def sigmoid_loss(self, logits, target, w_bce, w_dice, w_iou=0.0, w_jaccard=0.0, w_focal=0.0, w_lovasz=0.0):
        if logits.C != 1:
            raise StpShapeError("binary loss expects one class")
        if self.dry:
            return
        self.loss_scalars = self._alloc((16,), torch.float32)
        self.loss_scalars.zero_()
        count = logits.rows
        if w_iou or w_jaccard or w_focal:
            dl = self._emit_loss("stp_sigmoid_loss_ex", logits, target, (count,), (w_bce, w_dice, w_iou, w_jaccard, w_focal))
        else:
            dl = self._emit_loss("stp_sigmoid_bce_dice", logits, target, (count,), (w_bce, w_dice))
        logits.meta["loss_bias_grad"] = bool(self.training and not w_lovasz and self.dls is None)
        if w_lovasz:
            if self.training and self.loss_scale != 1.0:
                raise StpShapeError("lovasz_loss has no loss-scaling form: use loss_scale=1 (or bf16) with it")
            nbytes = int(self.lib.stp_lovasz_workspace_bytes(count, self.N))
            if nbytes <= 0:
                raise StpShapeError("lovasz_loss: the sort workspace cannot be sized (no device)")
            self.ws_lovasz = torch.empty(nbytes, dtype=torch.uint8, device=self.device)
            self._emit(self.fwd, "stp_lovasz_hinge", logits.buf.data_ptr(), target.buf.data_ptr(), self.N, count // self.N, self.cdt,
                       float(w_lovasz), self.loss_scalars.data_ptr(), dl.data_ptr() if dl is not None else None, logits.gradC,
                       self.ws_lovasz.data_ptr(), nbytes)
        logits.grad_ready = self.training

    def sigmoid_multilabel_loss(self, logits, target, w_bce, w_dice, w_iou=0.0, w_jaccard=0.0, w_focal=0.0):
        if not 2 <= logits.C <= 8:
            raise StpShapeError("multi-label loss expects 2..8 classes")
        if self.dry:
            return
        self.loss_scalars = self._alloc((16,), torch.float32)
        self.loss_scalars.zero_()
        self._emit_loss("stp_sigmoid_multilabel_loss", logits, target, (logits.rows, logits.C, logits.C), (w_bce, w_dice, w_iou, w_jaccard, w_focal))
        logits.meta["loss_bias_grad"] = "multilabel" if (self.training and self.dls is None) else False
        logits.grad_ready = self.training

    def softmax_loss(self, logits, target, w_cce, w_dice, w_iou=0.0, w_jaccard=0.0, w_focal=0.0):
        if logits.C < 2:
            raise StpShapeError("categorical loss expects at least two classes")
        if self.dry:
            return
        opts = self.masked_loss or {}
        ignore_label, class_weights = opts.get("ignore_label"), opts.get("class_weights")
        masked = ignore_label is not None or class_weights is not None
        if masked or w_iou or w_jaccard or w_focal:
            name, tail, ign = "stp_softmax_loss_ex", (), None
            if masked:
                if logits.C > 32:
                    raise StpShapeError("ignore_label / class_weights need a head of 2..32 classes")
                ign = -1 if ignore_label is None else int(ignore_label)
                cw = None
                if class_weights is not None:
                    if len(class_weights) != logits.C:
                        raise StpShapeError("class_weights: %d weights for %d classes" % (len(class_weights), logits.C))
                    cw = self._alloc((logits.C,), torch.float32)
                    cw.copy_(torch.tensor([float(w) for w in class_weights], dtype=torch.float32))
                self.class_weights = cw
                name, tail = "stp_softmax_loss_masked", (ign, cw.data_ptr() if cw is not None else None)
            self.loss_scalars = self._alloc((16,), torch.float32)
            self.loss_scalars.zero_()
            self._emit_loss(name, logits, target, (logits.rows, logits.C, logits.C), (w_cce, w_dice, w_iou, w_jaccard, w_focal), tail=tail)
            self._emit_confusion(logits, target, ignore_label=ign)
            logits.grad_ready = self.training
            return
        self.loss_scalars = self._alloc((12,), torch.float32)
        rec = logits.meta.get("resize_rec")
        if (self.training and rec is not None and self.fwd[rec[0]][2] == "stp_resize_bilinear" and rec[1].needs_grad
                and not rec[1].grad_ready and target.buf.data_ptr() % 4 == 0
                and self.lib.stp_softmax_cce_dice_up_ok(rec[2], logits.C, self.cdt)
                and (not self.class_metrics or self.lib.stp_class_confusion_up_ok(rec[2], logits.C, self.cdt))):
            idx, lo, f = rec
            logits.meta["deferred"] = (self.fwd[idx][0], self.fwd[idx][1], self.fwd[idx][2])
            self.fwd[idx] = (None, (), "fused:resize->loss", None)
            nb = int(self.lib.stp_softmax_cce_dice_up_corner_bytes(self.N, lo.H, lo.W, logits.C))
            corners = self._alloc((nb // 4,), torch.float32)
            dlow = self._gradbuf(lo)
            dls = self.dls.data_ptr() if self.dls is not None else None
# ... 167 lines not shown
            st = pl._alloc((max(nfl, 4),), torch.float32)
            p.stats_partial = st.data_ptr()
            out.meta["stats_table"] = pl._group_stats(p, st, Cout)
        self.flops = 2.0 * pl.N * self.Ho * self.Wo * Cout * k * k * self.Cin_master / (4.0 if self.transpose else 1.0)
        if flops_as is not None:
            self.flops = float(flops_as)
        pl._emit_conv(pl.fwd, p, {"layer": self.name, "pass": "fwd", "flops": self.flops, "tile": int(pl.lib.stp_conv2d_tile_for(C.byref(p))),
                                  "src2": bool(self.C1 or self.upsample)})

    def _weight_copies(self):
        pl, w, Cout, k, KWp, Cinp, Cin_master, param_cols = self.plan, self.w, self.Cout, self.k, self.KWp, self.Cinp, self.Cin_master, self.param_cols
        wf = self.wf = pl._alloc((_rup(Cout, 16) * k * KWp * Cinp,))
        self.need_dgrad = pl.training and (self.x_ng or self.s_ng) and not self.stem
        wb = self.wb = pl._alloc((_rup(Cinp, 16) * k * k * self.CoutB,)) if self.need_dgrad else None
        self.out.meta["wb"] = wb
        wsrc = pl._pptr(w)
        if param_cols is not None:
            w.pending_slices += 1
            wm = pl._alloc((Cout * Cin_master,), torch.float32)
            pl._emit(pl.prep, "stp_copy_cols_f32", wm.data_ptr(), Cin_master, wsrc + 4 * int(param_cols[0]), int(param_cols[1]), Cout, Cin_master, 0)
            wsrc = wm.data_ptr()
        self.out.meta["w_master"] = (wsrc, Cout, Cin_master, k)
        pl._prep_layers.append((wsrc, wf.data_ptr(), wb.data_ptr() if wb is not None else None, Cout, k, k, Cin_master, KWp, Cinp, self.CoutB))

    def _collapsed_copies(self):
        pl, p, C0, C1, rows_f = self.plan, self.p, self.C0, self.C1, _rup(self.Cout, 16)
        self.w4 = None
        if not (self.upsample and self.src1 is not None and self.k == 3 and self.KWp == 3 and self.stride == 1 and self.pad == 1
                and self.Cinp == self.Cin_master == C0 + C1
                and os.environ.get("STP_UPCOLLAPSE", "1") != "0" and not pl.lib.stp_conv2d_scn_eligible(C.byref(p))
                and int(pl.lib.stp_conv2d_halo_variant(C.byref(p))) < 0):
            return
        wup = pl._alloc((rows_f * 16 * C0,))
        pl._upc_layers.append((pl._pptr(self.w), wup.data_ptr(), self.Cout, rows_f, C0, C0 + C1))
        p.weight_up = wup.data_ptr()
        if self.need_dgrad and self.x_ng and C0 % 16 == 0 and os.environ.get("STP_UPCOLLAPSE_BWD", "0") == "1":
            self.w4 = pl._alloc((C0 * 16 * self.CoutB,))
            pl._upc4_layers.append((pl._pptr(self.w), self.w4.data_ptr(), self.Cout, self.CoutB, C0, C0 + C1))

    def _register_bn_consumer(self):
        pl, x, p, wp, w = self.plan, self.x, self.p, self.wp, self.w
        if not pl.training or x.meta.get("apply_rec") is None or self.src1 is not None or self.transpose or self.stem:
            return
        if self.residual is None and pl.lib.stp_conv2d_sc_eligible(C.byref(p)) and (not w.trainable or pl.lib.stp_wgrad_sc_eligible(C.byref(wp))):
            x.meta["sc_consumers"].append((p, wp))
        elif pl.fuse_bn_halo and not self.upsample and pl.lib.stp_conv2d_halo_variant(C.byref(p)) >= 0:
            x.meta["halo_consumers"].append((p, wp, (not w.trainable) or int(pl.lib.stp_conv2d_wgrad_kernel_id(C.byref(wp))) in (2, 3)))

    def backward(self):
        pl, out, residual, b = self.plan, self.out, self.residual, self.b
        if not out.needs_grad or not out.grad_ready:
            return
        dy = self.dy = out.grad
        if self.relu:
            pl._guard_write(dy)
            pl._emit(pl.bwd, "stp_relu_bwd", out.buf.data_ptr(), dy.data_ptr(), out.rows * out.gradC, pl.cdt)
        if residual is not None and residual.needs_grad:
            if not residual.grad_ready and residual.gradC == out.gradC:
                residual.grad = dy
                residual.grad_ready = True
            else:
                pl._emit(pl.bwd, "stp_add_inplace", pl._gradbuf(residual).data_ptr(), dy.data_ptr(), out.rows * out.gradC, pl.cdt)
        if self.w.trainable:
            self._weight_grad()
        if b is not None and b.trainable and out.meta.get("loss_bias_grad") and self.Cout == 1:
            pl._emit(pl.bwd, "stp_sigmoid_loss_bias_grad", pl.ws_loss.data_ptr(), out.rows, pl._gptr(b), 0)
        elif b is not None and b.trainable and out.meta.get("loss_bias_grad") == "multilabel":
            pl._emit(pl.bwd, "stp_sigmoid_multilabel_bias_grad", pl.ws_loss.data_ptr(), out.rows, self.Cout, pl._gptr(b), 0)
        elif b is not None and b.trainable:
            pl._emit_bias_grad(dy, out.rows, self.CoutB, self.Cout, b)
        if self.need_dgrad and not out.meta.get("dgrad_folded"):
            self._data_grad()

    def _weight_grad(self):
        pl, x, src1, w, wp, k, Cout, Cin_master, param_cols = self.plan, self.x, self.src1, self.w, self.wp, self.k, self.Cout, self.Cin_master, self.param_cols
        padded, gcols = self.stem or self.CoutB != Cout, None
        if padded:
            dwp = pl._alloc((self.CoutB * k * self.KWp * self.Cinp,), torch.float32)
            wp.dw = dwp.data_ptr()
        elif param_cols is not None:
            gcols = pl._alloc((Cout * Cin_master,), torch.float32)
            wp.dw = gcols.data_ptr()
        else:
            wp.dw = pl._gptr(w)
        wp.src0, wp.src1, wp.dy = x.meta.get("src_override") or x.buf.data_ptr(), (src1.buf.data_ptr() if src1 is not None else None), self.dy.data_ptr()
        cls = int(pl.lib.stp_wgrad_group_class(C.byref(wp))) if (pl.wgrad_group_gflop > 0 and not padded and gcols is None) else 0
        if cls:
            self._wgrad_join_group(cls)
        else:
            pl._flush_wgroup()
            pl._emit_wgrad(wp, self.name, self.flops, defer_hi=0 if (padded or gcols is not None) else w.end)
        if gcols is not None:
            w.pending_slices -= 1
            gbase = pl._gptr(w) if w.pending_slices == 0 else pl.G.data_ptr() + 4 * w.offset
            pl._emit(pl.bwd, "stp_copy_cols_f32", gbase + 4 * int(param_cols[0]), int(param_cols[1]), gcols.data_ptr(), Cin_master, Cout, Cin_master, 0)
        if padded:
            pl._emit(pl.bwd, "stp_weight_grad_unpad", dwp.data_ptr(), pl._gptr(w), Cout, k, k, Cin_master, self.KWp, self.Cinp, 0)
        beta = x.meta.get("input_bn_beta")
        if self.stem and beta is not None and beta.trainable:
            pl._emit(pl.bwd, "stp_stem_beta_grad", dwp.data_ptr(), pl._pptr(w), pl._gptr(beta), Cout, k, k, self.real_c0, self.KWp, self.Cinp, self.real_c0)

    def _wgrad_join_group(self, cls):
        pl = self.plan
        if pl._wgroup and pl._wgroup_cls != cls:
            pl._flush_wgroup()
        pl._wgroup.append((self.wp, self.name, self.flops))
        pl._wgroup_cls = cls
        pl._wgroup_flops += self.flops
        pl._wgroup_hi = max(pl._wgroup_hi, self.w.end)
        pl._wgroup_reads.add(self.dy.data_ptr())
        if pl._wgroup_flops >= pl.wgrad_group_gflop * 1e9:
            pl._flush_wgroup()

    def _data_grad(self):
        pl, x = self.plan, self.x
        self._dgrad_dests()
        q = self._dgrad_plain()
        if self.stride not in (1, 2):
            raise StpShapeError("data gradient supports stride 1 and 2")
        if self._form_scatter():
            return
        form = (self._form_s2d() or self._form_parity_fold(q) or self._form_fold1(q) or self._form_collapsed()
                or self._form_sum2x2_stream(q) or self._form_sum2x2_halo(q) or Dgrad(q, self))
        if form.folded_up and self.d0_hires is not None:
            pl._keep = [t for t in pl._keep if t is not self.d0_hires]
            self.d0 = self.d0_hires = None
        self._attach_bn_sums(form)
        pl._emit_conv(pl.bwd, form.q, {"layer": self.name, "pass": "dgrad", "flops": form.flops,
                                       "tile": int(pl.lib.stp_conv2d_tile_for(C.byref(form.q))), "s2d": form.s2d, "fold1": form.fold1})
        if self.upsample and self.x_ng and not form.folded_up:
            acc = int(x.grad_ready)
            pl._emit_grad_pass("stp_upsample2x_bwd", x, acc, (pl.N, x.H, x.W, self.C0, self.C0, pl.cdt),
                               (self.d0.data_ptr(), pl._gradbuf(x).data_ptr(), pl.N, x.H, x.W, self.C0, self.C0, pl.cdt, acc),
                               os.environ.get("STP_FUSE_UP_BN", "1") != "0")
        if self.x_ng:
            x.grad_ready = True
        if self.s_ng:
            self.src1.grad_ready = True

    def _dgrad_dests(self):
        pl, x, src1, shape = self.plan, self.x, self.src1, (self.plan.N, self.Hv, self.Wv)
        self.d0_hires = None
        if self.upsample:
            d0 = self.d0_hires = pl._alloc(shape + (self.C0,)) if self.x_ng else None
            self.acc0 = 0
        else:
            d0 = pl._gradbuf(x) if self.x_ng else None
            self.acc0 = int(x.grad_ready)
        d1 = pl._gradbuf(src1) if self.s_ng else None
        self.acc1 = int(src1.grad_ready) if self.s_ng else 0
        if d0 is None:
            d0 = pl._alloc(shape + (self.C0,))
        if self.C1 and d1 is None:
            d1 = pl._alloc(shape + (self.C1,))
        self.d0, self.d1 = d0, d1

    def _dgrad_plain(self):
        pl, x, k, stride, Ho, Wo, C0 = self.plan, self.x, self.k, self.stride, self.Ho, self.Wo, self.C0
        if self.transpose:
            return ops.conv_params(self.dy, self.wb, self.d0, N=pl.N, Hs0=Ho, Ws0=Wo, Hv=Ho, Wv=Wo, C0=self.CoutB, mode=ops.SRC_DIRECT, KH=k, KW=k,
                                   stride=2, pad=k - 1 - self.pad, Ho=x.H, Wo=x.W, Cout=C0, dtype=pl.cdt, accumulate0=self.acc0)
        return ops.conv_params(self.dy, self.wb, self.d0, N=pl.N, Hs0=Ho, Ws0=Wo,
                               Hv=(2 * Ho - 1 if stride == 2 else Ho), Wv=(2 * Wo - 1 if stride == 2 else Wo),
                               C0=self.CoutB, mode=(ops.SRC_ZEROINS2X if stride == 2 else ops.SRC_DIRECT), KH=k, KW=k, stride=1,
                               pad=k - 1 - self.pad, Ho=self.Hv, Wo=self.Wv, Cout=C0 + self.C1, dtype=pl.cdt, dst1=self.d1, Cd0=C0,
                               accumulate0=self.acc0, accumulate1=self.acc1)

    def _form_scatter(self):
        pl, x, N, Ho, Wo, C0 = self.plan, self.x, self.plan.N, self.Ho, self.Wo, self.C0
        if not (self.stride == 2 and self.k == 1 and self.pad == 0 and not self.transpose and not self.upsample and self.src1 is None and self.x_ng
                and self.fs is None and C0 % 4 == 0 and os.environ.get("STP_SCATTER_1X1S2", "1") != "0"):
            return False
        t_low = pl._alloc((N, Ho, Wo, C0))
        qg = ops.conv_params(self.dy, self.wb, t_low, N=N, Hs0=Ho, Ws0=Wo, Hv=Ho, Wv=Wo, C0=self.CoutB, mode=ops.SRC_DIRECT, KH=1, KW=1,
                             stride=1, pad=0, Ho=Ho, Wo=Wo, Cout=C0, dtype=pl.cdt)
        pl._emit_conv(pl.bwd, qg, {"layer": self.name, "pass": "dgrad", "flops": 2.0 * N * Ho * Wo * self.Cout * self.Cin_master,
                                   "tile": int(pl.lib.stp_conv2d_tile_for(C.byref(qg)))})
        pl._emit_grad_pass("stp_scatter2x_bwd", x, self.acc0, (N, x.H, x.W, C0, pl.cdt),
                           (t_low.data_ptr(), self.d0.data_ptr(), N, x.H, x.W, C0, pl.cdt, self.acc0))
        x.grad_ready = True
        return True

    def _sibling_ready(self):
        fs = self.fs
        return (fs is not None and self.src1 is None and self.x_ng and not self.transpose and fs.needs_grad and fs.grad_ready
                and fs.meta.get("wb") is not None and (fs.H, fs.W) == (self.Ho, self.Wo))

    def _fold_sibling(self):
        self.fs.meta["dgrad_folded"] = True
        self.x.grad_writes += 1

    def _form_s2d(self):
# ... 95 lines not shown
```

### segmentation_training_pipeline_amd/ops.py

```python
import ctypes as C

import torch

from . import _lib
from ._lib import BF16, F16, F32, U8, SRC_DIRECT, SRC_NEAREST2X, SRC_ZEROINS2X

_DT = {torch.float32: F32, torch.bfloat16: BF16, torch.float16: F16, torch.uint8: U8}


def dt(t):
    return _DT[t.dtype]


def ptr(t):
    return None if t is None else t.data_ptr()


def stream():
    return torch.cuda.current_stream().cuda_stream


def _dev(t):
    if t is not None and not t.is_cuda:
        raise _lib.StpError("tensor must live on the GPU (no CPU fallback)")
# ... 73 lines not shown
    def reduce(self):
        _lib.check(_lib.load().stp_wgrad_group_reduce(C.addressof(self.host), self.dev.data_ptr(), self.ws.data_ptr(), stream()), "stp_wgrad_group_reduce")

    def run(self):
        self.partial()
        self.reduce()


def wgrad_group_class(p):
    return int(_lib.load().stp_wgrad_group_class(C.byref(p)))


def weight_prepare(master, fwd, bwd, Cout, KH, KW, Cin, KWp, Cinp, CoutB, dtype):
    _lib.call("stp_weight_prepare", ptr(master), ptr(fwd), ptr(bwd), Cout, KH, KW, Cin, KWp, Cinp, CoutB, dtype, stream())


def weight_grad_unpad(padded, grad, Cout, KH, KW, Cin, KWp, Cinp, accumulate=0):
    _lib.call("stp_weight_grad_unpad", ptr(padded), ptr(grad), Cout, KH, KW, Cin, KWp, Cinp, accumulate, stream())


def stem_beta_grad(padded_dw, master, dbeta, Cout, KH, KW, Cin, KWp, Cinp, one_ch):
    _lib.call("stp_stem_beta_grad", ptr(padded_dw), ptr(master), ptr(dbeta), Cout, KH, KW, Cin, KWp, Cinp, one_ch, stream())


def bn_workspace_bytes(Cn):
    return int(_lib.load().stp_bn_workspace_bytes(Cn))


def bn_stats(x, rows, Cn, eps, momentum, mean, rstd, moving_mean, moving_var, workspace):
    _lib.call("stp_bn_stats", ptr(_dev(x)), dt(x), rows, Cn, eps, momentum, ptr(mean), ptr(rstd), ptr(moving_mean),
              ptr(moving_var), ptr(workspace), workspace.numel() * workspace.element_size(), stream())


def bn_apply(x, y, rows, Cn, Cy, mean, rstd, gamma, beta, relu, pad_value=0.0):
    _lib.call("stp_bn_apply", ptr(x), dt(x), ptr(y), dt(y), rows, Cn, Cy, ptr(mean), ptr(rstd), ptr(gamma), ptr(beta),
              int(relu), float(pad_value), stream())


def bn_inference(x, y, rows, Cn, Cy, mm, mv, eps, gamma, beta, relu, pad_value=0.0):
    _lib.call("stp_bn_inference", ptr(x), dt(x), ptr(y), dt(y), rows, Cn, Cy, ptr(mm), ptr(mv), float(eps), ptr(gamma),
              ptr(beta), int(relu), float(pad_value), stream())


def bn_backward(x, dy, dx, rows, Cn, mean, rstd, gamma, beta, dgamma, dbeta, relu, accumulate_dx, workspace):
    _lib.call("stp_bn_backward", ptr(x), ptr(dy), ptr(dx), dt(x), rows, Cn, ptr(mean), ptr(rstd), ptr(gamma), ptr(beta),
              ptr(dgamma), ptr(dbeta), int(relu), int(accumulate_dx), ptr(workspace),
              workspace.numel() * workspace.element_size(), stream())


def bn_backward_fused(x, g, dx, rows, Cn, mean, rstd, gamma, partial, tiles, dgamma, dbeta, accumulate_dx, workspace):
    _lib.call("stp_bn_backward_fused", ptr(x), ptr(g), ptr(dx), dt(x), rows, Cn, ptr(mean), ptr(rstd), ptr(gamma), ptr(partial),
              int(tiles), ptr(dgamma), ptr(dbeta), int(accumulate_dx), ptr(workspace),
              workspace.numel() * workspace.element_size(), stream())


def maxpool3x3s2(x, y, idx, N, H, W, Cn):
    _lib.call("stp_maxpool3x3s2", ptr(x), ptr(y), ptr(idx), N, H, W, Cn, dt(x), stream())


def maxpool3x3s2_bwd(idx, dy, dx, N, H, W, Cn, accumulate=0):
    _lib.call("stp_maxpool3x3s2_bwd", ptr(idx), ptr(dy), ptr(dx), N, H, W, Cn, dt(dy), int(accumulate), stream())


def maxpool2x2(x, y, idx, N, H, W, Cn):
    _lib.call("stp_maxpool2x2", ptr(x), ptr(y), ptr(idx), N, H, W, Cn, dt(x), stream())


def maxpool2x2_bwd(idx, dy, dx, N, H, W, Cn, accumulate=0):
    _lib.call("stp_maxpool2x2_bwd", ptr(idx), ptr(dy), ptr(dx), N, H, W, Cn, dt(dy), int(accumulate), stream())


def maxpool_k(x, y, idx, N, H, W, Cn, k):
    _lib.call("stp_maxpool_k", ptr(x), ptr(y), ptr(idx), N, H, W, Cn, k, dt(x), stream())


def maxpool_k_bwd(idx, dy, dx, N, H, W, Cn, k, accumulate=0):
    _lib.call("stp_maxpool_k_bwd", ptr(idx), ptr(dy), ptr(dx), N, H, W, Cn, k, dt(dy), int(accumulate), stream())


def relu_bwd(y, dy, count):
    _lib.call("stp_relu_bwd", ptr(y), ptr(dy), count, dt(dy), stream())


def zero_bytes(t, nbytes):
    _lib.call("stp_zero_bytes", ptr(t), nbytes, stream())


def resize_nearest(x, y, N, H, W, Cn, factor, ldo, coff):
    _lib.call("stp_resize_nearest", ptr(x), ptr(y), N, H, W, Cn, factor, ldo, coff, dt(x), stream())


def resize_nearest_bwd(dy, dx, N, H, W, Cn, factor, ldo, coff, accumulate=0):
    _lib.call("stp_resize_nearest_bwd", ptr(dy), ptr(dx), N, H, W, Cn, factor, ldo, coff, dt(dy), int(accumulate), stream())


def dropout_spatial(x, y, N, HW, Cn, rate, state, salt):
    _lib.call("stp_dropout_spatial", ptr(x), ptr(y), N, HW, Cn, float(rate), ptr(state), int(salt), dt(x), stream())


def softmax_act(z, p, rows, classes, ldz, ldp):
    _lib.call("stp_softmax_act", ptr(z), ptr(p), rows, classes, ldz, ldp, dt(z), stream())


def softmax_act_bwd(p, dp, dz, rows, classes, ldp, ldg):
    _lib.call("stp_softmax_act_bwd", ptr(p), ptr(dp), ptr(dz), rows, classes, ldp, ldg, dt(p), stream())

# ... 400 lines not shown
```

Baseline: 2564 images/sec.

## Recompute one-channel head data gradient inside BatchNorm backward instead of materializing it

Result: no change. 2584 images/sec, median of 6 (+0.8%).

```diff
diff --git a/include/stp_hip.h b/include/stp_hip.h
--- a/include/stp_hip.h
+++ b/include/stp_hip.h
@@ -159,6 +159,9 @@
                               const float* mean, const float* rstd, const float* gamma, const float* partial, int32_t tiles,
                               float* dgamma, float* dbeta, int32_t accumulate_dx, void* workspace, size_t workspace_bytes,
                               void* stream);
+int stp_bn_backward_conv_recompute(const stp_conv_params* conv, const void* x, void* dx, int32_t dtype, int64_t rows, int32_t C,
+                                   const float* mean, const float* rstd, const float* gamma, const float* partial, int32_t tiles,
+                                   float* dgamma, float* dbeta, void* workspace, size_t workspace_bytes, void* stream);
 int stp_bn_stats(const void* x, int32_t xdtype, int64_t rows, int32_t C, float eps, float momentum,
                  float* mean, float* rstd, float* moving_mean, float* moving_var,
                  void* workspace, size_t workspace_bytes, void* stream);
diff --git a/segmentation_training_pipeline_amd/_lib.py b/segmentation_training_pipeline_amd/_lib.py
--- a/segmentation_training_pipeline_amd/_lib.py
+++ b/segmentation_training_pipeline_amd/_lib.py
@@ -107,6 +107,7 @@
     "stp_bn_finalize_apply_ok": (i32, [i32, i64, i32, i32]),
     "stp_bn_finalize_apply": (i32, [vp, i32, vp, vp, i32, i64, i32, f32, f32, vp, vp, vp, vp, vp, vp, i32, vp]),
     "stp_bn_backward_fused_add": (i32, [vp, vp, vp, vp, i32, i64, i32, vp, vp, vp, vp, i32, vp, vp, i32, vp, sz, vp]),
+    "stp_bn_backward_conv_recompute": (i32, [C.POINTER(ConvParams), vp, vp, i32, i64, i32, vp, vp, vp, vp, i32, vp, vp, vp, sz, vp]),
     "stp_maxpool3x3s2": (i32, [vp, vp, vp, i32, i32, i32, i32, i32, vp]),
     "stp_maxpool3x3s2_bwd": (i32, [vp, vp, vp, i32, i32, i32, i32, i32, i32, vp]),
     "stp_bn_apply_maxpool3x3s2": (i32, [vp, vp, vp, vp, i32, i32, i32, i32, i32, vp, vp, vp, vp, i32, vp]),
diff --git a/segmentation_training_pipeline_amd/csrc/bn_pool.hip b/segmentation_training_pipeline_amd/csrc/bn_pool.hip
--- a/segmentation_training_pipeline_amd/csrc/bn_pool.hip
+++ b/segmentation_training_pipeline_amd/csrc/bn_pool.hip
@@ -1090,6 +1090,13 @@
   sums[C + c] = (float)Q;
   if (dbeta) dbeta[c] = (float)S;
   if (dgamma) dgamma[c] = (float)Q;
+}
+
+int bn_bwd_finalize_tiles_launch(const float* partial, int tiles, int C, void* workspace, float** sums, float* dgamma, float* dbeta, hipStream_t s) {
+  *sums = (float*)workspace + (size_t)(BN_MAX_BLOCKS - 1) * 2 * C;
+  hipLaunchKernelGGL(bn_bwd_finalize_tiles_kernel, dim3(C), dim3(256), 0, s, partial, tiles, C, *sums, dgamma, dbeta);
+  STP_LAUNCH_CHECK();
+  return STP_OK;
 }
 
 extern "C" int stp_bn_backward_slots(const void* x, const void* g, void* dx, int32_t dtype, int64_t rows, int32_t C, const float* mean,
diff --git a/segmentation_training_pipeline_amd/csrc/conv_sc.h b/segmentation_training_pipeline_amd/csrc/conv_sc.h
--- a/segmentation_training_pipeline_amd/csrc/conv_sc.h
+++ b/segmentation_training_pipeline_amd/csrc/conv_sc.h
@@ -18,6 +18,8 @@
   int sum2;
   uint32_t src_bytes;
   BnBack pbn;
+  const float* bsums;
+  float inv_rows;
 };
 
 template <typename T> struct ScStageBn;
@@ -121,5 +123,7 @@
 int stem_wg_lean_blocks(int N, int Ho, int Wo);
 int stem_wg_lean_launch(const void* src, const void* dy, float* slabs, int N, int H, int W, int Ho, int Wo, hipStream_t s);
 
+int bn_bwd_finalize_tiles_launch(const float* partial, int tiles, int C, void* workspace, float** sums, float* dgamma, float* dbeta, hipStream_t s);
+
 int sc_lean_launch(const ScArgs& a, int cin, int dtype, hipStream_t s);
 int sc_wg_lean_launch(const ScWgArgs& a, int cin, int cout, int dtype, int blocks, hipStream_t s);
diff --git a/segmentation_training_pipeline_amd/csrc/conv_sc.hip b/segmentation_training_pipeline_amd/csrc/conv_sc.hip
--- a/segmentation_training_pipeline_amd/csrc/conv_sc.hip
+++ b/segmentation_training_pipeline_amd/csrc/conv_sc.hip
@@ -557,19 +557,28 @@
   }
 }
 
+static bool sc_head1_shape(const stp_conv_params* p) {
+  static const bool lean = !(getenv("STP_SC_LEAN") && atoi(getenv("STP_SC_LEAN")) == 0);
+  return lean && sc_stream_on() && p->dtype == STP_H16 && p->C0 == 1 && p->C1 == 0 && p->KH == 3 && p->KW == 3 && p->stride == 1 && p->pad == 1 &&
+         p->Cout == 16 && p->Cd0 == 16 && !p->residual && !p->bias && !p->relu && p->Ho == p->Hv && p->Wo == p->Wv && p->Hs0 == p->Hv &&
+         p->Ws0 == p->Wv && (p->Wv & 7) == 0 && p->src0_mode == STP_SRC_DIRECT && p->bnb_x && !p->dst_sum2x2 && !p->stats_slots &&
+         !p->accumulate0 && !p->src_bn_mean;
+}
+
 extern "C" int stp_conv2d_sc_eligible(const stp_conv_params* p) {
   if (!p || !stp_dtype_ok(p->dtype)) return 0;
   const int vec = p->dtype == STP_H16 ? 8 : 4;
   const int cin = p->C0;
   const bool cin_ok = p->dtype == STP_F32 ? (cin == 4 || cin == 8 || cin == 16) : (cin == 8 || cin == 16 || cin == 32);
+  if (cin == 1) return sc_head1_shape(p);
   return p->KH == 3 && p->KW == 3 && p->stride == 1 && p->pad == 1 && p->C1 == 0 && cin_ok && (cin % vec) == 0 && p->Cout <= 32 &&
          p->Cd0 == p->Cout && !p->residual && p->Ho == p->Hv && p->Wo == p->Wv &&
          (p->src0_mode == STP_SRC_DIRECT || (p->src0_mode == STP_SRC_NEAREST2X && p->Hv == 2 * p->Hs0 && p->Wv == 2 * p->Ws0));
 }
 
-extern "C" int stp_conv2d_sc(const stp_conv_params* p, void* stream) {
-  if (!stp_conv2d_sc_eligible(p) || !p->src0 || !p->weight || !p->dst0) return STP_E_BADARG;
-  ScArgs a;
+static int sc_fill_args(const stp_conv_params* p, ScArgs& a) {
+  if (!stp_conv2d_sc_eligible(p) || !p->src0 || !p->weight || (!p->dst0 && p->C0 != 1)) return STP_E_BADARG;
+  a.bsums = nullptr; a.inv_rows = 0.f;
   a.src = (const char*)p->src0; a.weight = (const char*)p->weight; a.bias = p->bias; a.dst = (char*)p->dst0;
   a.N = p->N; a.H = p->Hv; a.W = p->Wv; a.Hs = p->Hs0; a.Ws = p->Ws0; a.Cout = p->Cout;
   a.up = p->src0_mode == STP_SRC_NEAREST2X; a.accumulate = p->accumulate0; a.relu = p->relu;
@@ -592,6 +601,13 @@
   if (a.pbn.mean && !a.pbn.rstd) return STP_E_BADARG;
   if (a.bnb.x && (!a.stats || !a.bnb.mean || !a.bnb.rstd || p->relu)) return STP_E_BADARG;
   if (a.sum2 && ((p->Cout & 3) || (a.H & 1) || (a.W & 1) || p->bias || p->relu || (a.stats && !a.bnb.x))) return STP_E_BADARG;
+  return STP_OK;
+}
+
+extern "C" int stp_conv2d_sc(const stp_conv_params* p, void* stream) {
+  ScArgs a;
+  const int rc = sc_fill_args(p, a);
+  if (rc != STP_OK) return rc;
   const_cast<stp_conv_params*>(p)->stats_tiles = stp_conv2d_sc_stats_tiles(p);
   hipStream_t s = (hipStream_t)stream;
   {
@@ -599,6 +615,26 @@
     if (r != 1) return r;
   }
   return p->dtype == STP_H16 ? dispatch_sc<bf16_t>(a, p->C0, s) : dispatch_sc<float>(a, p->C0, s);
+}
+
+extern "C" int stp_bn_backward_conv_recompute(const stp_conv_params* conv, const void* x, void* dx, int32_t dtype, int64_t rows, int32_t C,
+                                              const float* mean, const float* rstd, const float* gamma, const float* partial, int32_t tiles,
+                                              float* dgamma, float* dbeta, void* workspace, size_t workspace_bytes, void* stream) {
+  if (!conv || !x || !dx || !mean || !rstd || !partial || !workspace || tiles <= 0 || dtype != STP_H16 || conv->dtype != dtype) return STP_E_BADARG;
+  if (conv->C0 != 1 || conv->Cout != C || (int64_t)conv->N * conv->Hv * conv->Wv != rows || conv->bnb_x != x || conv->bnb_mean != mean ||
+      conv->bnb_rstd != rstd || conv->bnb_gamma != gamma)
+    return STP_E_BADARG;
+  if (workspace_bytes < stp_bn_workspace_bytes(C)) return STP_E_WORKSPACE;
+  ScArgs a;
+  int rc = sc_fill_args(conv, a);
+  if (rc != STP_OK) return rc;
+  hipStream_t s = (hipStream_t)stream;
+  float* sums = nullptr;
+  rc = bn_bwd_finalize_tiles_launch(partial, tiles, C, workspace, &sums, dgamma, dbeta, s);
+  if (rc != STP_OK) return rc;
+  a.dst = (char*)dx; a.stats = nullptr; a.bsums = sums; a.inv_rows = (float)(1.0 / (double)rows);
+  rc = sc_lean_launch(a, 1, dtype, s);
+  return rc == 1 ? STP_E_BADARG : rc;
 }
 
 struct ScwArgs {
@@ -1917,6 +1953,12 @@
   const int vec = p->dtype == STP_H16 ? 8 : 4;
   const bool c0ok = p->C0 == 16 || p->C0 == 32 || (p->C0 == 64 && vec == 8);
   const bool c1ok = p->C1 == 0 || p->C1 == 16 || p->C1 == 32 || (p->C1 == 64 && vec == 8);
+  if (p->Cout == 1) {
+    static const bool lean = !(getenv("STP_SC_LEAN") && atoi(getenv("STP_SC_LEAN")) == 0);
+    return lean && sc_stream_on() && vec == 8 && p->KH == 3 && p->KW == 3 && p->stride == 1 && p->pad == 1 && (p->C0 == 16 || p->C0 == 32) && p->C1 == 0 &&
+           p->Ho == p->Hv && p->Wo == p->Wv && p->Hs0 == p->Hv && p->Ws0 == p->Wv && (p->Wv & 7) == 0 && p->src0_mode == STP_SRC_DIRECT &&
+           (uint64_t)p->N * p->Hv * p->Wv * p->C0 * 2 < 0x80000000ull;
+  }
   return p->KH == 3 && p->KW == 3 && p->stride == 1 && p->pad == 1 && c0ok && c1ok &&
          (p->Cout == 8 || p->Cout == 16 || p->Cout == 32 || (p->Cout == 4 && vec == 4)) && (p->Cout % vec) == 0 &&
          p->Ho == p->Hv && p->Wo == p->Wv &&
diff --git a/segmentation_training_pipeline_amd/csrc/conv_sc_lean.hip b/segmentation_training_pipeline_amd/csrc/conv_sc_lean.hip
--- a/segmentation_training_pipeline_amd/csrc/conv_sc_lean.hip
+++ b/segmentation_training_pipeline_amd/csrc/conv_sc_lean.hip
@@ -1,6 +1,8 @@
 #include "conv_sc.h"
 
-enum { SCL_STATS = 0, SCL_BNB = 1, SCL_BNB_SUM2 = 2, SCL_HEAD = 3 };
+enum { SCL_STATS = 0, SCL_BNB = 1, SCL_BNB_SUM2 = 2, SCL_HEAD = 3, SCL_BNB_SUMS = 4, SCL_BNB_APPLY = 5 };
+
+constexpr int SC1_HW = SC_TW + 16, SC1_VPR = SC1_HW / 8;
 
 struct TileC { int n, y0, x0; bool interior; };
 
@@ -15,14 +17,20 @@
 template <int CIN, int TM, int EPI, bool PBN, bool UP>
 __global__ __launch_bounds__(256, (TM == 1 ? (CIN <= 16 ? SC_WPE_SMALL : 3) : 2)) void conv_sc_lean_kernel(const ScArgs a) {
   typedef bf16_t T;
-  constexpr int SZ = 2, VEC = 8, KC = 32, K = 9 * CIN, NCH = (K + KC - 1) / KC, VPP = CIN / VEC, PIXB = CIN * SZ;
-  constexpr int HH = UP ? SC_TH / 2 + 2 : SC_HH, HW = UP ? SC_TW / 2 + 2 : SC_HW;
-  constexpr int NV = HH * HW * VPP, NPASS = (NV + 255) / 256, BUF = NPASS * 4096;
+  constexpr bool ONE = CIN == 1;
+  constexpr int CK = ONE ? 8 : CIN;
+  constexpr int SZ = 2, VEC = 8, KC = 32, K = 9 * CK, NCH = (K + KC - 1) / KC, VPP = ONE ? 1 : CIN / VEC, PIXB = CIN * SZ;
+  constexpr int HH = UP ? SC_TH / 2 + 2 : SC_HH, HW = UP ? SC_TW / 2 + 2 : ONE ? SC1_HW : SC_HW;
+  constexpr int NV = ONE ? HH * SC1_VPR : HH * HW * VPP, NPASS = (NV + 255) / 256, BUF = NPASS * 4096;
+  constexpr int HX0 = ONE ? 8 : 1;
+  constexpr bool BNBF = EPI == SCL_BNB || EPI == SCL_BNB_SUMS || EPI == SCL_BNB_APPLY;
   constexpr bool PART = (K % KC) != 0;
   constexpr int COUT = EPI == SCL_HEAD ? 1 : TM * 16;
   constexpr int CB = COUT * SZ;
   static_assert(EPI != SCL_HEAD || TM == 1, "head: one output channel");
   static_assert(!PBN || EPI == SCL_STATS || EPI == SCL_HEAD, "producer BatchNormalization: forward only");
+  static_assert(!ONE || (BNBF && TM == 1 && !UP), "one-channel source: the head's data gradient");
+  static_assert(ONE || (EPI != SCL_BNB_SUMS && EPI != SCL_BNB_APPLY), "the recomputed passes read the one-channel gradient");
 
   extern __shared__ __attribute__((aligned(16))) char smem[];
   float* red = reinterpret_cast<float*>(smem + 2 * BUF);
@@ -50,9 +58,9 @@
 #pragma unroll
   for (int p = 0; p < NPASS; ++p) {
     const int v = p * 256 + tid, pix = v / VPP;
-    const int hy = pix / HW, hx = pix - hy * HW;
+    const int hy = ONE ? v / SC1_VPR : pix / HW, hx = ONE ? (v - hy * SC1_VPR) * 8 : pix - hy * HW;
     hyx[p] = v < NV ? (hy << 16 | hx) : -1;
-    lo[p] = v < NV ? (uint32_t)(((hy - 1) * a.Ws + (hx - 1)) * PIXB + cvb) : 0x80000000u;
+    lo[p] = v < NV ? (uint32_t)(((hy - 1) * a.Ws + (hx - HX0)) * PIXB + cvb) : 0x80000000u;
   }
 
   auto decode = [&](int tile) -> TileC {
@@ -76,7 +84,7 @@
     } else {
 #pragma unroll
       for (int p = 0; p < NPASS; ++p) {
-        const int gy = (t.y0 >> sh) - 1 + (hyx[p] >> 16), gx = (t.x0 >> sh) - 1 + (hyx[p] & 0xffff);
+        const int gy = (t.y0 >> sh) - 1 + (hyx[p] >> 16), gx = (t.x0 >> sh) - HX0 + (hyx[p] & 0xffff);
         const bool ok = live && hyx[p] >= 0 && (unsigned)gy < (unsigned)a.Hs && (unsigned)gx < (unsigned)a.Ws;
         const uint32_t off = ok ? (uint32_t)((t.n * a.Hs + gy) * a.Ws + gx) * (uint32_t)PIXB + (uint32_t)cvb : 0x80000000u;
         inside |= ok ? (1u << p) : 0u;
@@ -95,11 +103,11 @@
 #pragma unroll
   for (int c = 0; c < NCH; ++c) {
     const int k0 = c * KC + lg * VEC;
-    const int tap = k0 / CIN, ch = k0 - tap * CIN;
+    const int tap = k0 / CK, ch = ONE ? 0 : k0 - tap * CK;
     const int kh = tap / 3, kw = tap - kh * 3;
 #pragma unroll
     for (int ar = 0; ar < NA; ++ar) {
-      const int prow = UP ? wave + ((ar + kh + 1) >> 1) : wave * 2 + kh, pcol = UP ? ((lr + kw + 1) >> 1) : kw + lr;
+      const int prow = UP ? wave + ((ar + kh + 1) >> 1) : wave * 2 + kh, pcol = UP ? ((lr + kw + 1) >> 1) : kw + lr + (HX0 - 1);
       bla[ar][c] = (uint32_t)(uintptr_t)smem + ((k0 < K) ? (uint32_t)(((prow * HW + pcol) * CIN + ch) * SZ) : 0u);
     }
 #pragma unroll
@@ -118,7 +126,7 @@
   }
   f32x2 ksc[TM][2], ksh[TM][2];
   float alo = 0.f, ahi = 0.f;
-  if constexpr (EPI == SCL_BNB || EPI == SCL_BNB_SUM2) {
+  if constexpr (BNBF || EPI == SCL_BNB_SUM2) {
 #pragma unroll
     for (int i = 0; i < TM; ++i) {
       const BnBackCh k = bnback_load(a.bnb, TM == 2 ? lg * 8 + i * 4 : i * 16 + lg * 4);
@@ -127,6 +135,13 @@
     }
     alo = a.bnb.relu ? __uint_as_float(1u) : -__builtin_inff();
     ahi = a.bnb.relu == 2 ? __uint_as_float(0x40bfffffu) : __builtin_inff();
+  }
+  f32x4 asc = {0.f, 0.f, 0.f, 0.f}, amu = asc, ars = asc, ak1 = asc, ak2 = asc;
+  if constexpr (EPI == SCL_BNB_APPLY) {
+    const BnBackCh k = bnback_load(a.bnb, lg * 4);
+    asc = k.sc; amu = k.mu; ars = k.rs;
+    ak1 = *reinterpret_cast<const f32x4*>(a.bsums + lg * 4) * a.inv_rows;
+    ak2 = *reinterpret_cast<const f32x4*>(a.bsums + COUT + lg * 4) * a.inv_rows;
   }
   float bias0 = 0.f;
   if constexpr (EPI == SCL_HEAD) bias0 = a.bias ? a.bias[0] : 0.f;
@@ -141,7 +156,7 @@
 
   const bool own = !(lr & 1);
   auto prefetch = [&](const TileC& pt, const bool EDGE, u32x2 (&xo)[TM][4]) __attribute__((always_inline)) {
-    if constexpr (EPI == SCL_BNB) {
+    if constexpr (BNBF) {
       const char* xb = a.bnb.x + (((size_t)pt.n * a.H + pt.y0) * a.W + pt.x0) * CB;
 #pragma unroll
       for (int f = 0; f < 4; ++f) {
@@ -171,7 +186,7 @@
     }
   };
   u32x2 xp[TM][4];
-  constexpr bool AHEAD = (EPI == SCL_BNB || EPI == SCL_BNB_SUM2) && !(CIN == 32 && TM == 2 && EPI == SCL_BNB);
+  constexpr bool AHEAD = (BNBF || EPI == SCL_BNB_SUM2) && !(CIN == 32 && TM == 2 && EPI == SCL_BNB);
   if constexpr (AHEAD) {
     if (tc.interior) prefetch(tc, false, xp); else prefetch(tc, true, xp);
   }
@@ -220,18 +235,21 @@
       constexpr int R = 4 * NCH;
       constexpr int RING = (CIN == 32 && TM == 2 && EPI == SCL_BNB_SUM2) ? 4 : SC_RING;
       constexpr int D = RING < R ? RING : R;
-      u32x4 ring[D];
+      std::conditional_t<ONE, uint32_t, u32x4> ring[D];
       auto issue = [&ring, &bla](auto kc) {
         constexpr int k = decltype(kc)::value, F = k / NCH, c = k % NCH;
-        constexpr int OFF = UP ? (F & 1) * 8 * PIXB : ((F >> 1) * SC_HW + (F & 1) * 16) * PIXB;
-        asm volatile("ds_read_b128 %0, %1 offset:%2" : "=v"(ring[k % D]) : "v"(bla[UP ? (F >> 1) : 0][c]), "n"(OFF));
+        constexpr int OFF = UP ? (F & 1) * 8 * PIXB : ((F >> 1) * HW + (F & 1) * 16) * PIXB;
+        if constexpr (ONE) asm volatile("ds_read_u16 %0, %1 offset:%2" : "=v"(ring[k % D]) : "v"(bla[0][c]), "n"(OFF));
+        else asm volatile("ds_read_b128 %0, %1 offset:%2" : "=v"(ring[k % D]) : "v"(bla[UP ? (F >> 1) : 0][c]), "n"(OFF));
       };
       sc_unroll<D>(issue);
       sc_unroll<R>([&ring, &fa, &acc, &issue, last_ok](auto kc) {
         constexpr int k = decltype(kc)::value, F = k / NCH, c = k % NCH;
         constexpr int young = (R - 1 - k) < (D - 1) ? (R - 1 - k) : (D - 1);
         asm volatile("s_waitcnt lgkmcnt(%1)" : "+v"(ring[k % D]) : "n"(young));
-        u32x4 v = ring[k % D];
+        u32x4 v;
+        if constexpr (ONE) v = u32x4{ring[k % D], 0u, 0u, 0u};
+        else v = ring[k % D];
         if (PART && c == NCH - 1 && !last_ok) v = u32x4{0u, 0u, 0u, 0u};
 #pragma unroll
         for (int i = 0; i < TM; ++i) acc[i][F] = mfma16_16x16x32(fa[i][c], v, acc[i][F]);
@@ -273,7 +291,7 @@
           if (lg == 0 && okf[f]) *reinterpret_cast<T*>(of + so) = (T)(pack_bf16x2(x, 0.f) & 0xffffu);
         }
       }
-      if constexpr (EPI == SCL_BNB) {
+      if constexpr (BNBF) {
         char* ob = a.dst + (((size_t)t.n * a.H + t.y0) * a.W + t.x0) * CB;
 #pragma unroll
         for (int f = 0; f < 4; ++f) {
@@ -290,12 +308,24 @@
               const f32x2 tt = __builtin_elementwise_fma(xv, ksc[i][e], ksh[i][e]);
               const f32x2 g = {okf[f] && __builtin_amdgcn_fmed3f(tt.x, alo, ahi) == tt.x ? dy.x : 0.f,
                                okf[f] && __builtin_amdgcn_fmed3f(tt.y, alo, ahi) == tt.y ? dy.y : 0.f};
-              ss[i][2 * e] += g.x; ss[i][2 * e + 1] += g.y;
-              qq[i][2 * e] = fmaf(g.x, xv.x, qq[i][2 * e]); qq[i][2 * e + 1] = fmaf(g.y, xv.y, qq[i][2 * e + 1]);
-              o[e] = pack_bf16x2(g.x, g.y);
+              if constexpr (EPI == SCL_BNB_APPLY) {
+                float d[2];
+#pragma unroll
+                for (int u = 0; u < 2; ++u) {
+                  const int ch = 2 * e + u;
+                  const float gv = u ? g.y : g.x, xe = u ? xv.y : xv.x;
+                  const float xh = (xe - amu[ch]) * ars[ch];
+                  d[u] = asc[ch] * (gv - ak1[ch] - xh * ak2[ch]);
+                }
+                o[e] = pack_bf16x2(d[0], d[1]);
+              } else {
+                ss[i][2 * e] += g.x; ss[i][2 * e + 1] += g.y;
+                qq[i][2 * e] = fmaf(g.x, xv.x, qq[i][2 * e]); qq[i][2 * e + 1] = fmaf(g.y, xv.y, qq[i][2 * e + 1]);
+                o[e] = pack_bf16x2(g.x, g.y);
+              }
             }
           }
-          if (okf[f]) scl_store<TM>(of + so, oo);
+          if (EPI != SCL_BNB_SUMS && okf[f]) scl_store<TM>(of + so, oo);
         }
       }
       if constexpr (EPI == SCL_BNB_SUM2) {
@@ -344,8 +374,8 @@
     }
   }
 
-  if (EPI != SCL_HEAD && a.stats) {
-    if constexpr (EPI == SCL_BNB || EPI == SCL_BNB_SUM2) {
+  if (EPI != SCL_HEAD && EPI != SCL_BNB_APPLY && a.stats) {
+    if constexpr (BNBF || EPI == SCL_BNB_SUM2) {
 #pragma unroll
       for (int i = 0; i < TM; ++i) {
         const int cb = TM == 2 ? lg * 8 + i * 4 : i * 16 + lg * 4;
@@ -379,7 +409,7 @@
 template <int CIN, int TM, int EPI, bool PBN, bool UP>
 static int launch_scl(const ScArgs& a, hipStream_t s) {
   const int ntiles = a.N * a.tiles_x * a.tiles_y;
-  constexpr int NV = (UP ? (SC_TH / 2 + 2) * (SC_TW / 2 + 2) : SC_HH * SC_HW) * (CIN / 8), NPASS = (NV + 255) / 256;
+  constexpr int NV = CIN == 1 ? SC_HH * SC1_VPR : (UP ? (SC_TH / 2 + 2) * (SC_TW / 2 + 2) : SC_HH * SC_HW) * (CIN / 8), NPASS = (NV + 255) / 256;
   const size_t lds = (size_t)2 * NPASS * 4096 + (4 * TM * 16 * 2 + 64) * sizeof(float);
   const int blocks = sc_stream_blocks(STP_H16, CIN, TM * 16, ntiles);
   static bool attr_set = false;
@@ -422,6 +452,11 @@
   if (!sc_lean_on() || !sc_stream_on() || dtype != STP_H16 || a.stat_slots || a.accumulate || a.relu) return 1;
   const bool pbn = a.pbn.mean != nullptr;
   const int tm = a.Cout <= 16 ? 1 : 2;
+  if (cin == 1) {
+    if (!a.bnb.x || pbn || a.bias || a.sum2 || a.up || a.Cout != 16 || (a.W & 7) || (a.bsums ? !a.dst : !a.stats)) return STP_E_BADARG;
+    if (a.bsums) return launch_scl<1, 1, SCL_BNB_APPLY, false, false>(a, s);
+    return a.dst ? launch_scl<1, 1, SCL_BNB, false, false>(a, s) : launch_scl<1, 1, SCL_BNB_SUMS, false, false>(a, s);
+  }
   if (a.bnb.x) {
     if (pbn || a.bias || !a.stats || a.Cout != tm * 16) return 1;
     return a.sum2 ? dispatch_scl<SCL_BNB_SUM2, false>(a, cin, tm, s) : dispatch_scl<SCL_BNB, false>(a, cin, tm, s);
@@ -439,10 +474,11 @@
 __global__ __launch_bounds__(256) void conv_sc_wgrad_lean_kernel(const ScWgArgs a) {
   typedef bf16_t T;
   constexpr int SZ = 2, VEC = 8, TMo = (COUT + 15) / 16, TNi = CIN / 16, PIXB = CIN * SZ, DYB = COUT * SZ;
-  constexpr int VPPX = CIN / VEC, VPPD = COUT / VEC;
+  constexpr bool ONE = COUT == 1;
+  constexpr int VPPX = CIN / VEC, VPPD = ONE ? 1 : COUT / VEC;
   constexpr int HH = UP ? SC_TH / 2 + 2 : SC_HH, HW = UP ? SC_TW / 2 + 2 : SC_HW;
   constexpr int NVX = HH * HW * VPPX, NPX = (NVX + 255) / 256;
-  constexpr int NVD = SC_TH * SC_TW * VPPD, NPD = (NVD + 255) / 256;
+  constexpr int NVD = ONE ? SC_TH * SC_TW / 8 : SC_TH * SC_TW * VPPD, NPD = (NVD + 255) / 256;
   constexpr int XBUF = NPX * 4096, DBUF = NPD * 4096, BUF = XBUF + DBUF;
   constexpr int F3 = 3 * TMo * TNi;
   static_assert(4 * F3 * 1024 <= 2 * BUF, "the final reduction of a filter row fits the (dead) staging buffers");
@@ -485,7 +521,7 @@
     }
 #pragma unroll
     for (int p = 0; p < NPD; ++p) {
-      const int v = p * 256 + tid, pix = v / VPPD;
+      const int v = p * 256 + tid, pix = ONE ? v * 8 : v / VPPD;
       const int py = pix / SC_TW, px = pix % SC_TW;
       pyx[p] = v < NVD ? (py << 16 | px) : -1;
       lod[p] = v < NVD ? (uint32_t)((py * a.W + px) * DYB) + cvd : 0x80000000u;
@@ -537,7 +573,8 @@
     ScStageBn<T> sbn;
     if (PBN) sbn.load(a.pbn, (tid % VPPX) * VEC);
     const int xl = lg * 4 + (lr >> 2), qb = (lr & 3) * 8;
-    const uint32_t aA0 = (uint32_t)(uintptr_t)smem + (uint32_t)(XBUF + ((2 * wave * SC_TW + xl) * COUT) * SZ + qb);
+    const uint32_t aA0 = (uint32_t)(uintptr_t)smem + (ONE ? (uint32_t)(XBUF + (2 * wave * SC_TW + lg * 4) * SZ)
+                                                          : (uint32_t)(XBUF + ((2 * wave * SC_TW + xl) * COUT) * SZ + qb));
     uint32_t aB0[3];
 #pragma unroll
     for (int kw = 0; kw < 3; ++kw)
@@ -574,7 +611,8 @@
       u32x2 fb[2][3][TNi][2];
       sc_unroll<2 * TMo * 2>([&fa, aA](auto kc) {
         constexpr int k = decltype(kc)::value, r = k / (TMo * 2), i = (k / 2) % TMo, hl = k & 1;
-        asm volatile("ds_read_b64_tr_b16 %0, %1 offset:%2" : "=v"(fa[r][i][hl]) : "v"(aA), "n"((r * SC_TW * COUT + i * 16 + hl * 16 * COUT) * SZ));
+        if constexpr (ONE) asm volatile("ds_read_b64 %0, %1 offset:%2" : "=v"(fa[r][i][hl]) : "v"(aA), "n"((r * SC_TW + hl * 16) * SZ));
+        else asm volatile("ds_read_b64_tr_b16 %0, %1 offset:%2" : "=v"(fa[r][i][hl]) : "v"(aA), "n"((r * SC_TW * COUT + i * 16 + hl * 16 * COUT) * SZ));
       });
       auto issue_b = [&fb, &aB](auto hc) {
         constexpr int h = decltype(hc)::value;
@@ -648,7 +686,7 @@
 
 template <int CIN, int COUT, bool PBN, bool UP>
 static int launch_scwl(const ScWgArgs& a, int blocks, hipStream_t s) {
-  constexpr int NPX = ((UP ? (SC_TH / 2 + 2) * (SC_TW / 2 + 2) : SC_HH * SC_HW) * (CIN / 8) + 255) / 256, NPD = (SC_TH * SC_TW * (COUT / 8) + 255) / 256;
+  constexpr int NPX = ((UP ? (SC_TH / 2 + 2) * (SC_TW / 2 + 2) : SC_HH * SC_HW) * (CIN / 8) + 255) / 256, NPD = COUT == 1 ? 1 : (SC_TH * SC_TW * (COUT / 8) + 255) / 256;
   const size_t lds = (size_t)2 * (NPX + NPD) * 4096;
   static bool attr_set = false;
   if (lds > 64 * 1024 && !attr_set) {
@@ -669,6 +707,8 @@
 template <bool PBN, bool UP>
 static int dispatch_scwl(const ScWgArgs& a, int cin, int cout, int blocks, hipStream_t s) {
   switch (cin * 64 + cout) {
+    case 16 * 64 + 1: if constexpr (!UP) return (a.W & 7) ? STP_E_BADARG : launch_scwl<16, 1, PBN, UP>(a, blocks, s); else return 1;
+    case 32 * 64 + 1: if constexpr (!UP) return (a.W & 7) ? STP_E_BADARG : launch_scwl<32, 1, PBN, UP>(a, blocks, s); else return 1;
     case 16 * 64 + 8: return launch_scwl<16, 8, PBN, UP>(a, blocks, s);
     case 16 * 64 + 16: return launch_scwl<16, 16, PBN, UP>(a, blocks, s);
     case 16 * 64 + 32: return launch_scwl<16, 32, PBN, UP>(a, blocks, s);
diff --git a/segmentation_training_pipeline_amd/graph.py b/segmentation_training_pipeline_amd/graph.py
--- a/segmentation_training_pipeline_amd/graph.py
+++ b/segmentation_training_pipeline_amd/graph.py
@@ -94,6 +94,7 @@
         self.fuse_bn_backward = os.environ.get("STP_FUSE_BN_BACKWARD", "1") != "0"
         self.fuse_bn_backward_last = os.environ.get("STP_FUSE_BN_BACKWARD_LAST", "1") != "0"
         self.fold_upsample_grad = os.environ.get("STP_FOLD_UPSAMPLE_GRAD", "1") != "0"
+        self.head_recompute = os.environ.get("STP_HEAD_RECOMPUTE", "1") != "0"
         self.wgrad_group_gflop = float(os.environ.get("STP_WGRAD_GROUP_GFLOP", "300"))
         self.wgrad_lone_group_gflop = float(os.environ.get("STP_WGRAD_LONE_GROUP_GFLOP", "600"))
         self.reduce_batch = int(os.environ.get("STP_WGRAD_REDUCE_BATCH", "0"))
@@ -506,6 +507,7 @@
             self._emit(self.fwd, "stp_bn_apply", x.buf.data_ptr(), self.cdt, out.buf.data_ptr(), self.cdt, x.rows, Cn, Cn,
                        mean.data_ptr(), rstd.data_ptr(), gp, self._pptr(beta), int(relu), 0.0)
         out.meta["bn"] = (x.buf.data_ptr(), mean.data_ptr(), rstd.data_ptr(), gp, self._pptr(beta), int(relu))
+        out.meta["bn_input"] = x
         if self.fuse_bn_sc and slots is None:
             out.meta["apply_rec"] = self.fwd[-1]
             out.meta["sc_consumers"], out.meta["halo_consumers"] = [], []
@@ -519,7 +521,14 @@
                     and out.meta.get("bnb") is not None):
                 dadd, x.grad = x.grad, None
             dx = self._gradbuf(x) if x.needs_grad else self._alloc((x.N, x.H, x.W, Cn))
-            if bslots is not None:
+            if out.meta.get("bnb_recompute") is not None:
+                st, q = out.meta["bnb_recompute"]
+                if x.grad_ready and x.needs_grad:
+                    raise StpShapeError("%s: the recomputed BatchNormalization backward does not accumulate" % name)
+                self._emit(self.bwd, "stp_bn_backward_conv_recompute", C.byref(q), x.buf.data_ptr(), dx.data_ptr(), self.cdt, x.rows, Cn,
+                           mean.data_ptr(), rstd.data_ptr(), gp, st.data_ptr(), int(self.lib.stp_conv2d_stats_floats(C.byref(q))) // (2 * Cn),
+                           self._gptr(gamma) if gamma else None, self._gptr(beta), self.ws_bn.data_ptr(), self.ws_bn.numel() * 4)
+            elif bslots is not None:
                 self._emit(self.bwd, "stp_bn_backward_slots", x.buf.data_ptr(), out.grad.data_ptr(), dx.data_ptr(), self.cdt, x.rows, Cn,
                            mean.data_ptr(), rstd.data_ptr(), gp, bslots[0], bslots[1], self._gptr(gamma) if gamma else None,
                            self._gptr(beta), int(x.grad_ready and x.needs_grad))
@@ -587,6 +596,7 @@
         if self.dry:
             return L.out
         L.forward(bn_stats, flops_as)
+        L.out.meta["conv_layer"] = L
         if self.training:
             self._tape.append(L.backward)
         return L.out
@@ -1151,6 +1161,9 @@
         self.loss_scalars = self._alloc((16,), torch.float32)
         self.loss_scalars.zero_()
         count = logits.rows
+        if self._head_recompute_rule(logits, w_lovasz):
+            logits.gradC = 1
+            logits.meta["head_recompute"] = True
         if w_iou or w_jaccard or w_focal:
             dl = self._emit_loss("stp_sigmoid_loss_ex", logits, target, (count,), (w_bce, w_dice, w_iou, w_jaccard, w_focal))
         else:
@@ -1167,6 +1180,26 @@
                        float(w_lovasz), self.loss_scalars.data_ptr(), dl.data_ptr() if dl is not None else None, logits.gradC,
                        self.ws_lovasz.data_ptr(), nbytes)
         logits.grad_ready = self.training
+
+    HEAD_RECOMPUTE_MIN_ROWS = 256
+
+    def _head_recompute_rule(self, logits, w_lovasz):
+        L = logits.meta.get("conv_layer")
+        if not (self.head_recompute and self.training and self.dtype != "fp32" and L is not None and not w_lovasz and self.dls is None):
+            return False
+        x = L.x
+        bnm, pre = x.meta.get("bn"), x.meta.get("bn_input")
+        if not (L.Cout == 1 and L.k == 3 and L.stride == 1 and L.pad == 1 and L.src1 is None and L.residual is None and not L.upsample
+                and not L.transpose and not L.relu and not L.stem and L.fs is None and L.param_cols is None and L.CoutB == 8
+                and bnm is not None and pre is not None and x.meta.get("uses", 0) == 1 and pre.meta.get("uses", 0) == 1
+                and x.needs_grad and self.fuse_bn_backward and self.slot_arena is None and x.H >= self.HEAD_RECOMPUTE_MIN_ROWS
+                and self.lib.stp_conv2d_sc_eligible(C.byref(L.p))):
+            return False
+        q = L.dgrad_head1(None)
+        self._set_bnb(q, bnm)
+        w1 = _lib.WgradParams.from_buffer_copy(L.wp)
+        w1.Cout = 1
+        return bool(self.lib.stp_conv2d_sc_eligible(C.byref(q)) and (not L.w.trainable or self.lib.stp_wgrad_sc_eligible(C.byref(w1))))
 
     def sigmoid_multilabel_loss(self, logits, target, w_bce, w_dice, w_iou=0.0, w_jaccard=0.0, w_focal=0.0):
         if not 2 <= logits.C <= 8:
@@ -1440,6 +1473,7 @@
         if not out.needs_grad or not out.grad_ready:
             return
         dy = self.dy = out.grad
+        self.head1 = bool(out.meta.get("head_recompute"))
         if self.relu:
             pl._guard_write(dy)
             pl._emit(pl.bwd, "stp_relu_bwd", out.buf.data_ptr(), dy.data_ptr(), out.rows * out.gradC, pl.cdt)
@@ -1457,7 +1491,9 @@
             pl._emit(pl.bwd, "stp_sigmoid_multilabel_bias_grad", pl.ws_loss.data_ptr(), out.rows, self.Cout, pl._gptr(b), 0)
         elif b is not None and b.trainable:
             pl._emit_bias_grad(dy, out.rows, self.CoutB, self.Cout, b)
-        if self.need_dgrad and not out.meta.get("dgrad_folded"):
+        if self.need_dgrad and self.head1:
+            self._data_grad_head1()
+        elif self.need_dgrad and not out.meta.get("dgrad_folded"):
             self._data_grad()
 
     def _weight_grad(self):
@@ -1472,6 +1508,8 @@
         else:
             wp.dw = pl._gptr(w)
         wp.src0, wp.src1, wp.dy = x.meta.get("src_override") or x.buf.data_ptr(), (src1.buf.data_ptr() if src1 is not None else None), self.dy.data_ptr()
+        if self.head1:
+            wp.Cout = 1
         cls = int(pl.lib.stp_wgrad_group_class(C.byref(wp))) if (pl.wgrad_group_gflop > 0 and not padded and gcols is None) else 0
         if cls:
             self._wgrad_join_group(cls)
@@ -1526,6 +1564,22 @@
         if self.s_ng:
             self.src1.grad_ready = True
 
+    def dgrad_head1(self, dy):
+        pl = self.plan
+        return ops.conv_params(dy, self.wb, None, N=pl.N, Hs0=self.Ho, Ws0=self.Wo, Hv=self.Ho, Wv=self.Wo, C0=1, mode=ops.SRC_DIRECT, KH=3, KW=3,
+                               stride=1, pad=1, Ho=self.Hv, Wo=self.Wv, Cout=self.C0, dtype=pl.cdt)
+
+    def _data_grad_head1(self):
+        pl, x = self.plan, self.x
+        q = self.dgrad_head1(self.dy)
+        pl._set_bnb(q, x.meta["bn"])
+        st = pl._alloc((max(int(pl.lib.stp_conv2d_stats_floats(C.byref(q))), 4),), torch.float32)
+        q.stats_partial = st.data_ptr()
+        x.meta["bnb_recompute"] = (st, q)
+        pl._emit_conv(pl.bwd, q, {"layer": self.name, "pass": "dgrad", "flops": self.flops, "tile": int(pl.lib.stp_conv2d_tile_for(C.byref(q))),
+                                  "s2d": False, "fold1": False})
+        x.grad_ready = True
+
     def _dgrad_dests(self):
         pl, x, src1, shape = self.plan, self.x, self.src1, (self.plan.N, self.Hv, self.Wv)
         self.d0_hires = None
diff --git a/segmentation_training_pipeline_amd/ops.py b/segmentation_training_pipeline_amd/ops.py
--- a/segmentation_training_pipeline_amd/ops.py
+++ b/segmentation_training_pipeline_amd/ops.py
@@ -149,6 +149,11 @@
     _lib.call("stp_bn_backward_fused", ptr(x), ptr(g), ptr(dx), dt(x), rows, Cn, ptr(mean), ptr(rstd), ptr(gamma), ptr(partial),
               int(tiles), ptr(dgamma), ptr(dbeta), int(accumulate_dx), ptr(workspace),
               workspace.numel() * workspace.element_size(), stream())
+
+
+def bn_backward_conv_recompute(conv, x, dx, rows, Cn, mean, rstd, gamma, partial, tiles, dgamma, dbeta, workspace):
+    _lib.call("stp_bn_backward_conv_recompute", C.byref(conv), ptr(x), ptr(dx), dt(x), rows, Cn, ptr(mean), ptr(rstd), ptr(gamma),
+              ptr(partial), int(tiles), ptr(dgamma), ptr(dbeta), ptr(workspace), workspace.numel() * workspace.element_size(), stream())
 
 
 def maxpool3x3s2(x, y, idx, N, H, W, Cn):
```
